# WQCG/blitzdg

Hardware: AMD Instinct MI355X
Metric: element-DOF updates/sec (sw2d RHS + LSERK4 stage, N=4, 1M tris) (higher is better)
Workload: dtype f64

## Files before the change

### blitzdg_amd/_capi.py

```python
import ctypes
import os
from ctypes import (POINTER, Structure, byref, c_char_p, c_double, c_float, c_int, c_size_t, c_uint,
                    c_ulonglong, c_void_p)

import numpy as np

_HERE = os.path.dirname(os.path.abspath(__file__))
os.environ.setdefault("HSA_ENABLE_IPC_MODE_LEGACY", "0")
LIB_PATH = os.environ.get("BDG_HIP_LIBRARY") or os.path.join(_HERE, "lib", "libblitzdg_hip.so")

BDG_OK, BDG_ERR_ARGUMENT, BDG_ERR_RUNTIME, BDG_ERR_HIP, BDG_ERR_UNSTABLE = 0, 1, 2, 3, 4
BDG_F64, BDG_I32 = 0, 1
BDG_SW2D_REORDER = 1
BDG_SW2D_NODAL_GEOMETRY = 2
BDG_SW2D_KEEP_ORDER = 4
BDG_SW2DQ_GENERAL_GEOMETRY = 1
(FIELD_STATS_SUM, FIELD_STATS_ETA_MAX, FIELD_STATS_H_MIN, FIELD_STATS_SPEED_MAX, FIELD_STATS_COS, FIELD_STATS_SIN) = range(6)

(MESH_VERTICES, MESH_ELEMENTS, MESH_ETOE, MESH_ETOF, MESH_BCTYPE, MESH_EPART, MESH_NPART) = range(7)
(TRI_R, TRI_S, TRI_X, TRI_Y, TRI_V, TRI_VINV, TRI_DR, TRI_DS, TRI_DRW, TRI_DSW, TRI_LIFT, TRI_FILTER,
 TRI_J, TRI_RX, TRI_RY, TRI_SX, TRI_SY, TRI_NX, TRI_NY, TRI_FSCALE, TRI_FMASK, TRI_FX, TRI_FY,
 TRI_VMAPM, TRI_VMAPP, TRI_MAPP, TRI_VMAPB, TRI_MAPB, TRI_GATHER, TRI_SCATTER) = range(30)
(GAUSS_NX, GAUSS_NY, GAUSS_SJ, GAUSS_J, GAUSS_RX, GAUSS_RY, GAUSS_SX, GAUSS_SY, GAUSS_X, GAUSS_Y, GAUSS_W,
 GAUSS_INTERP, GAUSS_MAPM, GAUSS_MAPP) = range(14)
(CUB_R, CUB_S, CUB_WEIGHTS, CUB_V, CUB_RX, CUB_RY, CUB_SX, CUB_SY, CUB_J, CUB_DR, CUB_DS, CUB_MM, CUB_MMCHOL,
 CUB_X, CUB_Y, CUB_W) = range(16)
(N1D_R, N1D_X, N1D_V, N1D_VINV, N1D_DR, N1D_LIFT, N1D_J, N1D_RX, N1D_NX, N1D_FMASK, N1D_FX,
 N1D_FSCALE, N1D_ETOV, N1D_ETOE, N1D_ETOF, N1D_VMAPM, N1D_VMAPP) = range(17)


class BdgError(RuntimeError):

    def __init__(self, code, message):
        super().__init__(message)
        self.code = code


class NumericalInstability(BdgError):
    """BDG_ERR_UNSTABLE: the reference drivers throw 'A numerical instability has occurred!'."""


class Table(Structure):
    _fields_ = [("data", c_void_p), ("rows", c_int), ("cols", c_int), ("dtype", c_int)]


class Sw2dDesc(Structure):
    _fields_ = [("order", c_int), ("num_elements", c_int),
                ("Dr", c_void_p), ("Ds", c_void_p), ("Lift", c_void_p), ("Filter", c_void_p),
                ("rx", c_void_p), ("sx", c_void_p), ("ry", c_void_p), ("sy", c_void_p),
                ("nx", c_void_p), ("ny", c_void_p), ("Fscale", c_void_p),
                ("vmapM", c_void_p), ("vmapP", c_void_p), ("mapW", c_void_p), ("num_wall", c_int),
                ("g", c_double), ("device", c_int), ("flags", c_int),
                ("num_fields", c_int), ("sources", c_int), ("zx", c_void_p), ("zy", c_void_p),
                ("coriolis", c_void_p), ("coriolis_const", c_double), ("drag", c_double)]

# ... 203 lines not shown
    "bdg_quadnodes_bed_slopes": (c_int, [_P, _P, _P, _P]),
    "bdg_quadnodes_sponge_coeff": (c_int, [_P, _P, c_int, c_double, c_double, _P]),
    "bdg_quadnodes_quadrature_weights": (c_int, [_P, _P]),
    "bdg_quadnodes_locate_points": (c_int, [_P, _P, _P, c_int, _P, _P, _P]),
    "bdg_quadnodes_lagrange_basis": (c_int, [_P, _P, c_int, _P]),
    "bdg_sw2dq_enable_monitor": (c_int, [_P, POINTER(Sw2dqMonitorDesc)]),
    "bdg_sw2dq_monitor_sample": (c_int, [_P]),
    "bdg_sw2dq_monitor_count": (c_int, [_P, POINTER(c_int)]),
    "bdg_sw2dq_monitor_read": (c_int, [_P, c_int, c_int, _P]),
    "bdg_sw2dq_monitor_width": (c_int, [_P, POINTER(c_int)]),
    "bdg_sw2dq_monitor_reset": (c_int, [_P]),
    "bdg_sw2dq_monitor_reduce": (c_int, [_P]),
    "bdg_quadnodes_drifter_tables": (c_int, [_P, _P, c_int, _P, _P, _P]),
    "bdg_sw2dq_enable_drifters": (c_int, [_P, POINTER(Sw2dqDrifterDesc)]),
    "bdg_sw2dq_drifters_advance": (c_int, [_P, c_double, c_int]),
    "bdg_sw2dq_drifters_time": (c_int, [_P, c_double, c_int, POINTER(c_float)]),
    "bdg_sw2dq_drifters_state": (c_int, [_P, _P, _P, _P, _P, _P, _P]),
    "bdg_sw2dq_drifters_count": (c_int, [_P, POINTER(c_int), POINTER(c_int)]),
    "bdg_sw2dq_drifters_read": (c_int, [_P, c_int, c_int, _P, _P, _P, _P]),
    "bdg_sw2dq_drifters_reset": (c_int, [_P]),
    "bdg_sw2d_step_lserk4": (c_int, [_P, c_double, c_int]),
    "bdg_sw2d_lserk4_stages": (c_int, [_P, c_double, c_int]),
    "bdg_sw2d_step_rk2": (c_int, [_P, c_double, c_int, c_int]),
    "bdg_sw2d_step_ssprk2": (c_int, [_P, c_double, c_int, c_int, c_double]),
    "bdg_sw2d_compute_dt": (c_int, [_P, c_double, POINTER(c_double), POINTER(c_double)]),
    "bdg_sw2d_run_adaptive": (c_int, [_P, c_double, c_double, c_int, c_int, POINTER(c_double),
                                      POINTER(c_double), POINTER(c_int)]),
    "bdg_sw2d_set_partition": (c_int, [_P, c_int, c_int, _P, c_int]),
    "bdg_sw2d_halo_doubles_per_element": (c_int, [_P]),
    "bdg_sw2d_halo_pack": (c_int, [_P, _P]),
    "bdg_sw2d_halo_unpack": (c_int, [_P, _P]),
    "bdg_sw2d_lserk4_stage_part": (c_int, [_P, c_double, c_int]),
    "bdg_comm_unique_id": (c_int, [_P, c_int]),
    "bdg_sw2d_comm_init": (c_int, [_P, c_int, c_int, _P, _P, _P, _P, _P, _P, c_int]),
    "bdg_sw2d_lserk4_stages_exchanged": (c_int, [_P, c_double, c_int]),
    "bdg_sw2d_step_rk2_exchanged": (c_int, [_P, c_double, c_int, c_int]),
    "bdg_sw2d_step_ssprk2_exchanged": (c_int, [_P, c_double, c_int, c_int, c_double]),
    "bdg_sw2d_local_peers": (c_int, [_P, c_int, _P, _P, _P, _P, _P, c_int]),
    "bdg_sw2d_group_lserk4_stages": (c_int, [POINTER(_P), c_int, c_double, c_int]),
    "bdg_sw2d_compute_dt_global": (c_int, [_P, c_double, POINTER(c_double), POINTER(c_double)]),
    "bdg_sw2d_allreduce_max": (c_int, [_P, c_double, POINTER(c_double)]),
    "bdg_sw2d_allreduce_sum": (c_int, [_P, c_double, POINTER(c_double)]),
    "bdg_sw2d_barrier": (c_int, [_P]),
    "bdg_sw2d_rhs_resident": (c_int, [_P, _P, _P, _P]),
    "bdg_sw2d_synchronize": (c_int, [_P]),
    "bdg_sw2d_time_lserk4_stages": (c_int, [_P, c_double, c_int, POINTER(c_float)]),
    "bdg_probe_stream_triad": (c_int, [c_int, c_size_t, c_int, POINTER(c_double)]),
    "bdg_sw2d_probe_stage_traffic": (c_int, [_P, c_int, POINTER(c_float)]),
    "bdg_sw2d_uses_affine_geometry": (c_int, [_P]),
    "bdg_sw2d_is_renumbered": (c_int, [_P]),
    "bdg_element_order": (c_int, [_P, c_int, c_int, _P]),
    "bdg_element_order_wanted": (c_int, [_P, c_int, c_int]),
    "bdg_sw2d_device_bytes": (c_size_t, [_P]),
    "bdg_sw2d_stream": (c_void_p, [_P]),
    "bdg_trinodes_quadrature_weights": (c_int, [_P, _P]),
    "bdg_trinodes_locate_points": (c_int, [_P, _P, _P, c_int, _P, _P, _P]),
    "bdg_trinodes_interpolation_rows": (c_int, [_P, _P, _P, c_int, _P]),
    "bdg_sw2d_enable_monitor": (c_int, [_P, POINTER(Sw2dMonitorDesc)]),
    "bdg_sw2d_monitor_sample": (c_int, [_P]),
    "bdg_sw2d_monitor_count": (c_int, [_P, POINTER(c_int)]),
    "bdg_sw2d_monitor_read": (c_int, [_P, c_int, c_int, _P]),
    "bdg_sw2d_monitor_width": (c_int, [_P, POINTER(c_int)]),
    "bdg_sw2d_monitor_reset": (c_int, [_P]),
    "bdg_sw2d_monitor_reduce": (c_int, [_P]),
    "bdg_sw2d_monitor_time": (c_int, [_P, c_int, POINTER(c_float)]),
    "bdg_trinodes_drifter_tables": (c_int, [_P, _P, c_int, _P, _P, _P, _P]),
    "bdg_sw2d_enable_drifters": (c_int, [_P, POINTER(Sw2dDrifterDesc)]),
    "bdg_sw2d_drifters_advance": (c_int, [_P, c_double, c_int]),
    "bdg_sw2d_drifters_time": (c_int, [_P, c_double, c_int, POINTER(c_float)]),
    "bdg_sw2d_drifters_state": (c_int, [_P, _P, _P, _P, _P, _P, _P]),
    "bdg_sw2d_drifters_count": (c_int, [_P, POINTER(c_int), POINTER(c_int)]),
    "bdg_sw2d_drifters_read": (c_int, [_P, c_int, c_int, _P, _P, _P, _P]),
    "bdg_sw2d_drifters_reset": (c_int, [_P]),
    **{f"{_abi}_{_name}": _sig for _abi in ("bdg_sw2d", "bdg_sw2dq") for _name, _sig in {
        "enable_field_stats": (c_int, [_P, POINTER(FieldStatsDesc)]),
        "field_stats_sample": (c_int, [_P]),
        "field_stats_count": (c_int, [_P, POINTER(c_int), POINTER(c_int)]),
        "field_stats_read": (c_int, [_P, c_int, c_int, _P]),
        "field_stats_samples": (c_int, [_P, c_int, c_int, _P]),
        "field_stats_reset": (c_int, [_P]),
        "field_stats_time": (c_int, [_P, c_int, POINTER(c_float)]),
    }.items()},
    "bdg_sw2d_curved_create": (c_int, [POINTER(Sw2dCurvedDesc), POINTER(_P)]),
    "bdg_sw2d_curved_plan": (c_int, [POINTER(Sw2dCurvedDesc), POINTER(c_int), c_int]),
    "bdg_sw2d_curved_destroy": (None, [_P]),
    "bdg_sw2d_curved_rhs": (c_int, [_P, _P, _P, _P, _P, _P, _P, _P, _P, c_int]),
    "bdg_sw2d_curved_set_state": (c_int, [_P, _P, _P, _P, _P]),
    "bdg_sw2d_curved_get_state": (c_int, [_P, _P, _P, _P, _P]),
    "bdg_sw2d_curved_step_rk2": (c_int, [_P, c_double, c_int, c_int]),
    "bdg_sw2d_curved_lserk4_stages": (c_int, [_P, c_double, c_int]),
    "bdg_sw2d_curved_time_rk2": (c_int, [_P, c_double, c_int, c_int, POINTER(c_float)]),
    "bdg_sw2d_curved_synchronize": (c_int, [_P]),
    "bdg_sw2d_curved_device_bytes": (c_size_t, [_P]),
    "bdg_sw2d_curved_bytes_per_element": (c_double, [_P]),
    "bdg_sw2d_curved_form": (c_int, [_P]),
    "bdg_sw2d_curved_kernel_info": (c_int, [_P, c_int, POINTER(c_int), c_int]),
    "bdg_sw2d_curved_get_elements": (c_int, [_P, c_int, c_int, c_int, POINTER(c_double)]),
    "bdg_sw2d_curved_set_elements": (c_int, [_P, c_int, c_int, c_int, POINTER(c_double)]),
    "bdg_sw2d_curved_rk2_phase": (c_int, [_P, c_double, c_int, c_int]),
    "bdg_sw2d_curved_set_partition": (c_int, [_P, c_int, c_int, _P, c_int]),
    "bdg_sw2d_curved_comm_init": (c_int, [_P, c_int, c_int, _P, _P, _P, _P, _P, _P, c_int]),
    "bdg_sw2d_curved_step_rk2_exchanged": (c_int, [_P, c_double, c_int, c_int]),
    "bdg_sw2d_curved_lserk4_stages_exchanged": (c_int, [_P, c_double, c_int]),
    "bdg_sw2d_curved_exchange": (c_int, [_P, c_int]),
    "bdg_sw2d_curved_barrier": (c_int, [_P]),
    "bdg_sw2d_curved_enable_driver": (c_int, [_P, POINTER(Sw2dCurvedDriverDesc)]),
# ... 55 lines not shown
```

### blitzdg_amd/csrc/hip/sw2d_affine_kernel.hpp

```cpp
#pragma once
#include "sw2d_kernels.hpp"

namespace bdg_dev {

template <int N>
struct AffineOps {
    using E = Elem<N>;
    static constexpr int OFF_D = 0;
    static constexpr int OFF_LIFT = 2 * E::Np * E::Np;
    static constexpr int DOUBLES = OFF_LIFT + E::NFN * E::Np;
};

__device__ __forceinline__ double fast_rcp(double x) {
    double r = __builtin_amdgcn_rcp(x);
    r = fma(fma(-x, r, 1.0), r, r);
    r = fma(fma(-x, r, 1.0), r, r);
    return r;
}

__device__ __forceinline__ double fast_sqrt(double x) {
    x = fmax(x, 1e-290);
    const double y = __builtin_amdgcn_rsq(x);
    double g = x * y, h = 0.5 * y;
    const double r = fma(-h, g, 0.5);
    g = fma(g, r, g);
    h = fma(h, r, h);
    g = fma(fma(-g, g, x), h, g);
    return g;
}

template <typename T>
__device__ __forceinline__ T ld_row(const T* row, unsigned byteOff) {
    return *reinterpret_cast<const T*>(reinterpret_cast<const char*>(row) + byteOff);
}
template <typename T>
__device__ __forceinline__ void st_row(T* row, unsigned byteOff, T v) {
    *reinterpret_cast<T*>(reinterpret_cast<char*>(row) + byteOff) = v;
}

struct PhysParams {
    const double* sx;
    const double* sy;
    const double* fcor;
    const double* fmat;
    double fconst, cd, slope, dragSign;
    const double* H;
    const int* obc;
    const double* lam;
    const double* spongeField;
    double tide;
};

template <int N>
__device__ __forceinline__ unsigned link_node(unsigned code, int n) {
    using E = Elem<N>;
    const bool rev = (code & 4u) != 0;
    const unsigned f = code & 3u;
    const unsigned m0 = rev ? E::fmask(0, N - n) : E::fmask(0, n);
    const unsigned m1 = rev ? E::fmask(1, N - n) : E::fmask(1, n);
    const unsigned m2 = rev ? E::fmask(2, N - n) : E::fmask(2, n);
    return f == 0u ? m0 : (f == 1u ? m1 : m2);
}

constexpr int STAGE_VMAP = -1;

template <int N, int MODE, int PHYS = 0, bool TRACER = false, bool SPONGE = false, int KIND = STAGE_VMAP>
__global__ __launch_bounds__(256) void sw2d_stage_affine_kernel(const StageParams p, const PhysParams ph) {
    using E = Elem<N>;
    constexpr int Np = E::Np, Nfp = E::Nfp, NFN = E::NFN;
    constexpr bool kLinks = KIND != STAGE_VMAP;
    static_assert(!kLinks || (MODE == MODE_LSERK && PHYS == 0 && !TRACER && !SPONGE), "face links: three-field LSERK stages");
    constexpr bool kReadRes = MODE == MODE_LSERK && KIND != STAGE_FIRST;
    constexpr bool kWriteRes = KIND != STAGE_LAST;

    const unsigned nwg = gridDim.x, xcd = blockIdx.x % 8u, q8 = nwg / 8u, r8 = nwg % 8u;
    const unsigned tile = (xcd < r8 ? xcd * (q8 + 1u) : r8 * (q8 + 1u) + (xcd - r8) * q8) + blockIdx.x / 8u;
    const unsigned k = static_cast<unsigned>(p.kbegin) + tile * blockDim.x + threadIdx.x;
    if (k >= static_cast<unsigned>(p.kend)) return;
    const unsigned k8 = k * 8u, k4 = k * 4u;

    const long long ld = p.ld, plane = static_cast<long long>(Np) * ld;
    const double* __restrict__ ops = p.opsAffine;
    const double* __restrict__ qin = p.qin;

    int idx[kLinks ? 1 : NFN];
    unsigned lnk[kLinks ? 3 : 1];
    if constexpr (kLinks) {
        const unsigned* __restrict__ fl = reinterpret_cast<const unsigned*>(p.faceLink);
#pragma unroll
        for (int f = 0; f < 3; ++f) lnk[f] = ld_row(fl + f * ld, k4);
    } else {
#pragma unroll
        for (int j = 0; j < NFN; ++j) idx[j] = ld_row(p.vmapP + j * ld, k4);
    }
    double h[Np], hu[Np], hv[Np], hN[TRACER ? Np : 1];
#pragma unroll
    for (int n = 0; n < Np; ++n) {
        h[n] = ld_row(qin + n * ld, k8);
        hu[n] = ld_row(qin + plane + n * ld, k8);
        hv[n] = ld_row(qin + 2 * plane + n * ld, k8);
        if constexpr (TRACER) hN[n] = ld_row(qin + 3 * plane + n * ld, k8);
    }
    const double* __restrict__ ag = p.ageo;
    const double rx = ld_row(ag, k8), sx = ld_row(ag + ld, k8), ry = ld_row(ag + 2 * ld, k8), sy = ld_row(ag + 3 * ld, k8);
    double fnx[3], fny[3], fsc[3];
#pragma unroll
    for (int f = 0; f < 3; ++f) {
        fnx[f] = ld_row(ag + (4 + f) * ld, k8);
        fny[f] = ld_row(ag + (7 + f) * ld, k8);
        fsc[f] = ld_row(ag + (10 + f) * ld, k8);
    }
    double ssx[PHYS != 0 ? Np : 1], ssy[PHYS != 0 ? Np : 1], sfc[PHYS != 0 ? Np : 1];
    if constexpr (PHYS != 0) {
#pragma unroll
        for (int i = 0; i < Np; ++i) { ssx[i] = 0.0; ssy[i] = 0.0; sfc[i] = ph.fconst; }
        if (ph.sx) {
#pragma unroll
            for (int i = 0; i < Np; ++i) ssx[i] = ld_row(ph.sx + i * ld, k8);
        }
        if (ph.sy) {
#pragma unroll
            for (int i = 0; i < Np; ++i) ssy[i] = ld_row(ph.sy + i * ld, k8);
        }
        if (ph.fcor) {
#pragma unroll
            for (int i = 0; i < Np; ++i) sfc[i] = ld_row(ph.fcor + i * ld, k8);
        }
    }
    __builtin_amdgcn_sched_barrier(0);
// ... 216 lines not shown
                n2 = a * old2[i] + dt * R2[i];
                n3 = a * old3[i] + dt * R3[i];
            } else if constexpr (kReadRes) {
                n1 = fma(dt, R1[i], a * old1[i]);
                n2 = fma(dt, R2[i], a * old2[i]);
                n3 = fma(dt, R3[i], a * old3[i]);
            } else {
                n1 = dt * R1[i];
                n2 = dt * R2[i];
                n3 = dt * R3[i];
            }
            if constexpr (kWriteRes) {
                st_row(rs + i * ld, k8, n1);
                st_row(rs + plane + i * ld, k8, n2);
                st_row(rs + 2 * plane + i * ld, k8, n3);
            }
            st_row(o + i * ld, k8, h[i] + b * n1);
            st_row(o + plane + i * ld, k8, hu[i] + b * n2);
            st_row(o + 2 * plane + i * ld, k8, hv[i] + b * n3);
            if constexpr (TRACER) {
                const double n4 = a * old4[i] + dt * R4[i];
                st_row(rs + 3 * plane + i * ld, k8, n4);
                st_row(o + 3 * plane + i * ld, k8, hN[i] + b * n4);
            }
        }
    } else {
        static_assert(!SPONGE || MODE == MODE_COMBINE, "the sponge follows a combine step");
        double* __restrict__ o = p.qout;
        const double a = p.ca, b = p.cb, c = p.cc;
        const double sg = p.sponge;
#pragma unroll
        for (int i = 0; i < Np; ++i) {
            const double v2 = a * old2[i] + b * hu[i] + c * R2[i], v3 = a * old3[i] + b * hv[i] + c * R3[i];
            st_row(o + i * ld, k8, a * old1[i] + b * h[i] + c * R1[i]);
            st_row(o + plane + i * ld, k8, SPONGE ? v2 / (1.0 + sg * v2 * v2) : v2);
            st_row(o + 2 * plane + i * ld, k8, SPONGE ? v3 / (1.0 + sg * v3 * v3) : v3);
        }
        if constexpr (TRACER) {
#pragma unroll
            for (int i = 0; i < Np; ++i) st_row(o + 3 * plane + i * ld, k8, a * old4[i] + b * hN[i] + c * R4[i]);
        }
    }
}

}

namespace bdg_dev {

template <int N, int MODE, int WAVES>
__global__ __launch_bounds__(256, WAVES) void sw2d_stage_affine_stream_kernel(const StageParams p) {
    using E = Elem<N>;
    constexpr int Np = E::Np, Nfp = E::Nfp;

    const unsigned nwg = gridDim.x, xcd = blockIdx.x % 8u, q8 = nwg / 8u, r8 = nwg % 8u;
    const unsigned tile = (xcd < r8 ? xcd * (q8 + 1u) : r8 * (q8 + 1u) + (xcd - r8) * q8) + blockIdx.x / 8u;
    const unsigned k = static_cast<unsigned>(p.kbegin) + tile * blockDim.x + threadIdx.x;
    if (k >= static_cast<unsigned>(p.kend)) return;
    const unsigned k8 = k * 8u, k4 = k * 4u;

    const long long ld = p.ld, plane = static_cast<long long>(Np) * ld;
    const double* __restrict__ ops = p.opsAffine;
    const double* __restrict__ qin = p.qin;
    const double* __restrict__ ag = p.ageo;
    const double g = p.g, halfg = 0.5 * p.g;

    double R1[Np], R2[Np], R3[Np];
#pragma unroll
    for (int i = 0; i < Np; ++i) R1[i] = R2[i] = R3[i] = 0.0;

    {
        const double rx = ld_row(ag, k8), sx = ld_row(ag + ld, k8), ry = ld_row(ag + 2 * ld, k8),
                     sy = ld_row(ag + 3 * ld, k8);
        constexpr int VCH = 5, NCH = (Np + VCH - 1) / VCH;
        double hc[2][VCH], huc[2][VCH], hvc[2][VCH];
#pragma unroll
        for (int t = 0; t < VCH; ++t)
            if (t < Np) {
                hc[0][t] = ld_row(qin + t * ld, k8);
                huc[0][t] = ld_row(qin + plane + t * ld, k8);
                hvc[0][t] = ld_row(qin + 2 * plane + t * ld, k8);
            }
#pragma unroll
        for (int c = 0; c < NCH; ++c) {
            const int cur = c & 1, nxt = cur ^ 1;
#pragma unroll
            for (int t = 0; t < VCH; ++t) {
                const int m = (c + 1) * VCH + t;
                if (m < Np) {
                    hc[nxt][t] = ld_row(qin + m * ld, k8);
                    huc[nxt][t] = ld_row(qin + plane + m * ld, k8);
                    hvc[nxt][t] = ld_row(qin + 2 * plane + m * ld, k8);
                }
            }
            __builtin_amdgcn_sched_barrier(0);
#pragma unroll
            for (int t = 0; t < VCH; ++t) {
                const int m = c * VCH + t;
                if (m < Np) {
                    const double h = hc[cur][t], hu = huc[cur][t], hv = hvc[cur][t];
                    const double r = fast_rcp(h);
                    const double u = hu * r, v = hv * r;
                    const double pr = halfg * h * h;
                    const double F2 = hu * u + pr, G2 = hu * v, G3 = hv * v + pr;
                    const double a1 = -(rx * hu + ry * hv), b1 = -(sx * hu + sy * hv);
                    const double a2 = -(rx * F2 + ry * G2), b2 = -(sx * F2 + sy * G2);
                    const double a3 = -(rx * G2 + ry * G3), b3 = -(sx * G2 + sy * G3);
#pragma unroll
                    for (int i = 0; i < Np; ++i) {
// ... 95 lines not shown
#pragma unroll
            for (int t = 0; t < CH; ++t) {
                const int i = i0 + t;
                if (i < Np) {
                    q1[t] = ld_row(qin + i * ld, k8);
                    q2[t] = ld_row(qin + plane + i * ld, k8);
                    q3[t] = ld_row(qin + 2 * plane + i * ld, k8);
                    o1[t] = ld_row(base2 + i * ld, k8);
                    o2[t] = ld_row(base2 + plane + i * ld, k8);
                    o3[t] = ld_row(base2 + 2 * plane + i * ld, k8);
                }
            }
            __builtin_amdgcn_sched_barrier(0);
#pragma unroll
            for (int t = 0; t < CH; ++t) {
                const int i = i0 + t;
                if (i < Np) {
                    if constexpr (MODE == MODE_LSERK) {
                        const double n1 = a * o1[t] + c * R1[i], n2 = a * o2[t] + c * R2[i], n3 = a * o3[t] + c * R3[i];
                        st_row(p.res + i * ld, k8, n1);
                        st_row(p.res + plane + i * ld, k8, n2);
                        st_row(p.res + 2 * plane + i * ld, k8, n3);
                        st_row(o + i * ld, k8, q1[t] + b * n1);
                        st_row(o + plane + i * ld, k8, q2[t] + b * n2);
                        st_row(o + 2 * plane + i * ld, k8, q3[t] + b * n3);
                    } else {
                        st_row(o + i * ld, k8, a * o1[t] + b * q1[t] + c * R1[i]);
                        st_row(o + plane + i * ld, k8, sponge_relax_no_test(a * o2[t] + b * q2[t] + c * R2[i], p.sponge));
                        st_row(o + 2 * plane + i * ld, k8, sponge_relax_no_test(a * o3[t] + b * q3[t] + c * R3[i], p.sponge));
                    }
                }
            }
            __builtin_amdgcn_sched_barrier(0);
        }
    }
}

}

namespace bdg_dev {

template <int N>
__device__ __forceinline__ int fmask_rt(int f, int n) {
    const int rs = n * (N + 1) - (n * (n - 1)) / 2;
    return f == 0 ? n : (f == 1 ? rs + (N - n) : rs);
}

template <int N, int MODE, int FIELDS>
__global__ __launch_bounds__(FIELDS == 3 ? 256 : 192, 2) void sw2d_stage_affine_rolled_kernel(const StageParams p) {
    using E = Elem<N>;
    constexpr int Np = E::Np, Nfp = E::Nfp;
    static_assert(FIELDS == 1 || FIELDS == 3, "FIELDS is 1 or 3");

    const unsigned nwg = gridDim.x, xcd = blockIdx.x % 8u, q8 = nwg / 8u, r8 = nwg % 8u;
    const unsigned tile = (xcd < r8 ? xcd * (q8 + 1u) : r8 * (q8 + 1u) + (xcd - r8) * q8) + blockIdx.x / 8u;
    const int c = FIELDS == 3 ? 0 : __builtin_amdgcn_readfirstlane(threadIdx.x >> 6);
    const unsigned k = static_cast<unsigned>(p.kbegin) +
                       (FIELDS == 3 ? tile * 256u + threadIdx.x : tile * 64u + (threadIdx.x & 63u));
    if (k >= static_cast<unsigned>(p.kend)) return;
    const unsigned k8 = k * 8u, k4 = k * 4u;

    const long long ld = p.ld, plane = static_cast<long long>(Np) * ld;
    const double* __restrict__ ops = p.opsAffine;
    const double* __restrict__ qin = p.qin;
    const double* __restrict__ ag = p.ageo;
    const double g = p.g, halfg = 0.5 * p.g;

    double R[FIELDS][Np];
#pragma unroll
    for (int q = 0; q < FIELDS; ++q)
#pragma unroll
        for (int i = 0; i < Np; ++i) R[q][i] = 0.0;

    {
        const double rx = ld_row(ag, k8), sx = ld_row(ag + ld, k8), ry = ld_row(ag + 2 * ld, k8),
                     sy = ld_row(ag + 3 * ld, k8);
        double h = ld_row(qin, k8), hu = ld_row(qin + plane, k8), hv = ld_row(qin + 2 * plane, k8);
#pragma unroll 1
        for (int m = 0; m < Np; ++m) {
            const int mn = m + 1 < Np ? m + 1 : m;
            const double hn = ld_row(qin + mn * ld, k8), hun = ld_row(qin + plane + mn * ld, k8),
                         hvn = ld_row(qin + 2 * plane + mn * ld, k8);
            const double r = fast_rcp(h);
            const double u = hu * r, v = hv * r;
            const double pr = halfg * h * h;
            const double F2 = hu * u + pr, G2 = hu * v, G3 = hv * v + pr;
            const double* __restrict__ row = ops + AffineOps<N>::OFF_D + 2 * m * Np;
            if constexpr (FIELDS == 3) {
                const double a1 = -(rx * hu + ry * hv), b1 = -(sx * hu + sy * hv);
                const double a2 = -(rx * F2 + ry * G2), b2 = -(sx * F2 + sy * G2);
                const double a3 = -(rx * G2 + ry * G3), b3 = -(sx * G2 + sy * G3);
#pragma unroll
                for (int i = 0; i < Np; ++i) {
                    const double dr = row[2 * i], ds = row[2 * i + 1];
                    R[0][i] = fma(ds, b1, fma(dr, a1, R[0][i]));
                    R[FIELDS - 2][i] = fma(ds, b2, fma(dr, a2, R[FIELDS - 2][i]));
                    R[FIELDS - 1][i] = fma(ds, b3, fma(dr, a3, R[FIELDS - 1][i]));
                }
            } else {
                const double F = c == 0 ? hu : (c == 1 ? F2 : G2);
                const double G = c == 0 ? hv : (c == 1 ? G2 : G3);
                const double a = -(rx * F + ry * G), b = -(sx * F + sy * G);
#pragma unroll
                for (int i = 0; i < Np; ++i) R[0][i] = fma(row[2 * i + 1], b, fma(row[2 * i], a, R[0][i]));
            }
            h = hn; hu = hun; hv = hvn;
        }
    }
// ... 101 lines not shown
```

### blitzdg_amd/csrc/hip/sw2d_affine_lean_kernel.hpp

```cpp
#pragma once
#include "sw2d_affine_kernel.hpp"

namespace bdg_dev {

template <int N>
__global__ __launch_bounds__(64, 2) void sw2d_stage_affine_lean_kernel(const StageParams p) {
    using E = Elem<N>;
    constexpr int Np = E::Np, Nfp = E::Nfp;

    const unsigned nwg = gridDim.x, xcd = blockIdx.x % 8u, q8 = nwg / 8u, r8 = nwg % 8u;
    const unsigned tile = (xcd < r8 ? xcd * (q8 + 1u) : r8 * (q8 + 1u) + (xcd - r8) * q8) + blockIdx.x / 8u;
    const unsigned k = static_cast<unsigned>(p.kbegin) + tile * blockDim.x + threadIdx.x;
    if (k >= static_cast<unsigned>(p.kend)) return;
    const unsigned k8 = k * 8u, k4 = k * 4u;

    const long long ld = p.ld, plane = static_cast<long long>(Np) * ld;
    const double* __restrict__ ops = p.opsAffine;
    const double* __restrict__ qin = p.qin;
    const double* __restrict__ ag = p.ageo;
    const double g = p.g, halfg = 0.5 * p.g;

    double h[Np], hu[Np], hv[Np];
#pragma unroll
    for (int n = 0; n < Np; ++n) {
        h[n] = ld_row(qin + n * ld, k8);
        hu[n] = ld_row(qin + plane + n * ld, k8);
        hv[n] = ld_row(qin + 2 * plane + n * ld, k8);
    }
    __builtin_amdgcn_sched_barrier(0);

    double R1[Np], R2[Np], R3[Np];
#pragma unroll
    for (int i = 0; i < Np; ++i) R1[i] = R2[i] = R3[i] = 0.0;

    {
        const double rx = ld_row(ag, k8), sx = ld_row(ag + ld, k8), ry = ld_row(ag + 2 * ld, k8), sy = ld_row(ag + 3 * ld, k8);
#pragma unroll
        for (int m = 0; m < Np; ++m) {
            const double r = fast_rcp(h[m]);
            const double u = hu[m] * r, v = hv[m] * r;
            const double pr = halfg * h[m] * h[m];
            const double F2 = hu[m] * u + pr, G2 = hu[m] * v, G3 = hv[m] * v + pr;
            const double a1 = -(rx * hu[m] + ry * hv[m]), b1 = -(sx * hu[m] + sy * hv[m]);
            const double a2 = -(rx * F2 + ry * G2), b2 = -(sx * F2 + sy * G2);
            const double a3 = -(rx * G2 + ry * G3), b3 = -(sx * G2 + sy * G3);
#pragma unroll
            for (int i = 0; i < Np; ++i) {
                const double dr = ops[AffineOps<N>::OFF_D + 2 * (m * Np + i)];
                R1[i] = fma(dr, a1, R1[i]);
                R2[i] = fma(dr, a2, R2[i]);
                R3[i] = fma(dr, a3, R3[i]);
            }
#pragma unroll
            for (int i = 0; i < Np; ++i) {
                const double ds = ops[AffineOps<N>::OFF_D + 2 * (m * Np + i) + 1];
                R1[i] = fma(ds, b1, R1[i]);
                R2[i] = fma(ds, b2, R2[i]);
                R3[i] = fma(ds, b3, R3[i]);
            }
        }
    }
    __builtin_amdgcn_sched_barrier(0);

#pragma unroll
// ... 89 lines not shown
```

### blitzdg_amd/csrc/hip/sw2d_affine_xchg_kernel.hpp

```cpp
#pragma once
#include "sw2d_affine_kernel.hpp"
#include "sw2d_mfma3_kernel.hpp"

namespace bdg_dev {

template <int N>
__global__ __launch_bounds__(64) void sw2d_stage_affine_xchg_kernel(const StageParams p, unsigned ldMagic) {
    using E = Elem<N>;
    constexpr int Np = E::Np, Nfp = E::Nfp, NFN = E::NFN;
    __shared__ double xs[3 * Np * 64];

    const unsigned nwg = gridDim.x, xcd = blockIdx.x % 8u, q8 = nwg / 8u, r8 = nwg % 8u;
    const unsigned tile = (xcd < r8 ? xcd * (q8 + 1u) : r8 * (q8 + 1u) + (xcd - r8) * q8) + blockIdx.x / 8u;
    const unsigned base = static_cast<unsigned>(p.kbegin) + tile * 64u, lane = threadIdx.x;
    const unsigned k = base + lane;
    if (k >= static_cast<unsigned>(p.kend)) return;
    const unsigned k8 = k * 8u, k4 = k * 4u;

    const long long ld = p.ld, plane = static_cast<long long>(Np) * ld;
    const unsigned ldu = static_cast<unsigned>(ld), planeBytes = static_cast<unsigned>(plane * 8);
    const double* __restrict__ ops = p.opsAffine;
    const double* __restrict__ qin = p.qin;
    const __amdgpu_buffer_rsrc_t rq = plane_rsrc(qin, 3u * planeBytes);

    int idx[NFN];
#pragma unroll
    for (int j = 0; j < NFN; ++j) idx[j] = ld_row(p.vmapP + j * ld, k4);
    double h[Np], hu[Np], hv[Np];
#pragma unroll
    for (int n = 0; n < Np; ++n) {
        h[n] = ld_row(qin + n * ld, k8);
        hu[n] = ld_row(qin + plane + n * ld, k8);
        hv[n] = ld_row(qin + 2 * plane + n * ld, k8);
    }
    const double* __restrict__ ag = p.ageo;
    const double rx = ld_row(ag, k8), sx = ld_row(ag + ld, k8), ry = ld_row(ag + 2 * ld, k8), sy = ld_row(ag + 3 * ld, k8);
    double fnx[3], fny[3], fsc[3];
#pragma unroll
    for (int f = 0; f < 3; ++f) {
        fnx[f] = ld_row(ag + (4 + f) * ld, k8);
        fny[f] = ld_row(ag + (7 + f) * ld, k8);
        fsc[f] = ld_row(ag + (10 + f) * ld, k8);
    }
    __builtin_amdgcn_sched_barrier(0);

    double hP[NFN], huP[NFN], hvP[NFN];
    unsigned ldsAt[NFN];
#pragma unroll
    for (int j = 0; j < NFN; ++j) {
        const unsigned o = static_cast<unsigned>(idx[j] < 0 ? -(idx[j] + 1) : idx[j]);
        unsigned nn = __umulhi(o, ldMagic);
        nn -= (nn * ldu > o) ? 1u : 0u;
        const unsigned kl = o - nn * ldu - base;
        const bool inwave = kl < 64u;
        ldsAt[j] = inwave ? nn * 64u + kl : 0xffffffffu;
        const unsigned o8 = inwave ? 0xfffffff8u : o * 8u;
        hP[j] = bld_f64(rq, o8, 0u);
        huP[j] = bld_f64(rq, o8, planeBytes);
        hvP[j] = bld_f64(rq, o8, 2u * planeBytes);
    }
    __builtin_amdgcn_sched_barrier(0);
#pragma unroll
    for (int n = 0; n < Np; ++n) {
        xs[n * 64 + lane] = h[n];
        xs[(Np + n) * 64 + lane] = hu[n];
        xs[(2 * Np + n) * 64 + lane] = hv[n];
// ... 121 lines not shown
```

### blitzdg_amd/csrc/hip/sw2d_device.hip

```cpp
#include "../host/capi_internal.hpp"
#include "../host/element_order.hpp"
#include "../host/parallel_for.hpp"
#include "blitzdg/LSERK4.hpp"
#include "run_records.hpp"
#include "sw2d_launch.hpp"
#include "sw2d_launch_host.hpp"
#include "sw2d_drifter_kernel.hpp"
#include <algorithm>
#include <atomic>
#include <cmath>
#include <cstdlib>
#include <cstring>
#include <limits>
#include <queue>
#include <stdexcept>
#include <string>
#include <vector>

namespace bdg_dev {

const KernelTable* kernel_table_order1();
const KernelTable* kernel_table_order2();
const KernelTable* kernel_table_order3();
const KernelTable* kernel_table_order4();
// ... 26 lines not shown
    for (int i = threadIdx.x; i < nblocks; i += blockDim.x) {
        const double x = part[2 * i], y = part[2 * i + 1];
        if (x != x || y != y) sBad = 1;
        a = fmax(a, x);
        b = fmax(b, y);
    }
    sA[threadIdx.x] = a;
    sB[threadIdx.x] = b;
    __syncthreads();
    for (int s = 128; s > 0; s >>= 1) {
        if (static_cast<int>(threadIdx.x) < s) {
            sA[threadIdx.x] = fmax(sA[threadIdx.x], sA[threadIdx.x + s]);
            sB[threadIdx.x] = fmax(sB[threadIdx.x], sB[threadIdx.x + s]);
        }
        __syncthreads();
    }
    if (threadIdx.x == 0) {
        const double nan = __builtin_nan("");
        out2[0] = sBad ? nan : sA[0];
        out2[1] = sBad ? nan : sB[0];
    }
}

template <typename T>
__global__ void scatter_rows_kernel(const T* __restrict__ src, T* __restrict__ dst, int rows, int K, long long ld,
                                    const int* __restrict__ perm) {
    const long long t = static_cast<long long>(blockIdx.x) * blockDim.x + threadIdx.x;
    if (t >= static_cast<long long>(rows) * K) return;
    const long long r = t / K, k = t % K;
    dst[r * ld + (perm ? perm[k] : k)] = src[t];
}

template <typename T>
__global__ void gather_rows_kernel(const T* __restrict__ src, T* __restrict__ dst, int rows, int K, long long ld,
                                   const int* __restrict__ perm) {
    const long long t = static_cast<long long>(blockIdx.x) * blockDim.x + threadIdx.x;
    if (t >= static_cast<long long>(rows) * K) return;
    const long long r = t / K, k = t % K;
    dst[t] = src[r * ld + (perm ? perm[k] : k)];
}

__global__ __launch_bounds__(256) void triad_kernel(double2* __restrict__ a, const double2* __restrict__ b,
                                                    const double2* __restrict__ c, double s, size_t n2) {
    const size_t stride = static_cast<size_t>(gridDim.x) * blockDim.x;
    for (size_t i = static_cast<size_t>(blockIdx.x) * blockDim.x + threadIdx.x; i < n2; i += stride) {
        const double2 x = b[i], y = c[i];
        a[i] = make_double2(x.x + s * y.x, x.y + s * y.y);
    }
}

__global__ __launch_bounds__(256) void stage_traffic_probe_kernel(const double* __restrict__ qin, double* __restrict__ qout,
                                                                 double* __restrict__ res, const double* __restrict__ ageo,
                                                                 const int* __restrict__ vmapP, int rows, int idxRows,
                                                                 long long ld, int K, int readRes, int writeRes) {
    const unsigned k = blockIdx.x * blockDim.x + threadIdx.x;
    if (k >= static_cast<unsigned>(K)) return;
    double acc = 0.0;
    for (int r = 0; r < 13; ++r) acc += ageo[r * ld + k];
    for (int r = 0; r < idxRows; ++r) acc += vmapP[r * ld + k];
    for (int r = 0; r < rows; ++r) {
        const double q = qin[r * ld + k], o = readRes ? res[r * ld + k] : 0.0;
        const double n = 0.5 * o + 1e-300 * (q + acc);
        if (writeRes) res[r * ld + k] = n;
        qout[r * ld + k] = q + 1e-300 * n;
    }
}

}

using bdg_detail::arg_error;
using bdg_detail::guard;
using bdg_detail::hip_error;
using bdg_detail::unstable_error;

using bdg_dev::DevBuf;
using bdg_dev::hipCheck;
using bdg_rccl::ncclCheck;
using bdg_rccl::rccl;

namespace {
std::vector<double> matmulHost(const double* A, const double* B, int n, int c);

namespace env {
int smallLaunchPinned() {
    static const int v = [] { const char* e = std::getenv("BDG_SW2D_SMALL_LAUNCH"); return e ? std::atoi(e) : -1; }();
    return v;
}
int interiorCapPinned() {
    static const int v = [] { const char* e = std::getenv("BDG_SW2D_INTERIOR_CAP"); return e ? std::atoi(e) : 0; }();
    return v;
}
bool extLaunch() {
    static const bool v = [] { const char* e = std::getenv("BDG_SW2D_EXT_LAUNCH"); return !e || e[0] != '0'; }();
    return v;
}
const char* affineVariantPin() { return std::getenv("BDG_SW2D_AFFINE_VARIANT"); }
bool nodalVector() { return std::getenv("BDG_SW2D_NODAL_VECTOR") != nullptr; }
bool fullStageTraffic() {
    const char* e = std::getenv("BDG_SW2D_FULL_STAGE_TRAFFIC");
    return e && e[0] != '0';
}
bool rolledSources() { return std::getenv("BDG_SW2D_ROLLED_SOURCES") != nullptr; }
bool eventFence() {
    const char* on = std::getenv("BDG_SW2D_EVENT_FENCE");
    const char* off = std::getenv("BDG_SW2D_EVENT_NOFENCE");
    return (on && on[0] == '1') || (off && off[0] == '0');
}
bool noCommWarmup() { return std::getenv("BDG_SW2D_NO_COMM_WARMUP") != nullptr; }
bool eventSync() {
    const char* e = std::getenv("BDG_SW2D_EVENT_SYNC");
    return e && e[0] != '0';
}
bool sourcesProduct() {
    const char* e = std::getenv("BDG_SW2D_SOURCES_PRODUCT");
    return e && e[0] != '0';
}
bool speedPass() { return std::getenv("BDG_SW2D_SPEED_PASS") != nullptr; }
bool tracerPass() { return std::getenv("BDG_SW2D_TRACER_PASS") != nullptr; }
bool sourcesTwoWave() { return std::getenv("BDG_SW2D_SOURCES_TWO_WAVE") != nullptr; }
bool haloKernels() { return std::getenv("BDG_SW2D_HALO_KERNELS") != nullptr; }
bool stripThroughput() { return std::getenv("BDG_SW2D_STRIP_THROUGHPUT") != nullptr; }
const char* haloVariant() { return std::getenv("BDG_SW2D_HALO_VARIANT"); }
}
}

struct bdg_sw2d {
    const bdg_dev::KernelTable* kt = nullptr;
    int N = 0, Np = 0, Nfp = 0, NFN = 0, K = 0, device = 0;
    long long ld = 0;
    double g = 9.81;
    bool hasFilter = false, hasH = false;
    hipStream_t stream = nullptr;
    size_t bytes = 0;
    DevBuf<double> qA, qB, res, aux, geo, fgeo, ops, Hbuf, stage, partials, red2;
    DevBuf<double> ageo, opsAffine, opsAffineFiltered;
    DevBuf<double> opsMfma, opsMfmaFiltered;
    DevBuf<double> opsMfma2, opsMfma2Filtered;
    DevBuf<double> opsMfma2Src, opsMfma2SrcFiltered;
    DevBuf<double> opsMfma2NodalFilter;
    bool mfmaSources = false;
    bool affine = false;
    bool nodalMfma = false;
    bool fastSources = false;
    static constexpr int kUnrolledSourcesMaxOrder = 4;
    DevBuf<double> filterT;
    int nf = 3;
    bool variantD = false;
    bdg_dev::VdParams vd{};
    DevBuf<double> zxBuf, zyBuf, fcorBuf, opsVd, opsVdFiltered;
    DevBuf<double> opsVn, filterRows, vnRaw;
    bool variantB = false;
    bdg_dev::VbParams vb{};
    DevBuf<double> HxBuf, HyBuf, spongeBuf, lamBuf, vbPartials;
    DevBuf<double> outM;
    DevBuf<int> obcBuf;
    double tideAmp = 0.0, tidePeriod = 1.0, tideRamp = 0.0;
    double timeNow = 0.0;
    bool lamExternal = false;
    DevBuf<double> lamPair;
    int lamSlot = 0;
    const double* lamStateFor = nullptr;
    double lamTideFor = 0.0;
    double nextEvalTime = 0.0;
    std::vector<double> hostDr, hostDs, hostLift, hostFilter, hostFDr, hostFDs, hostFLift;
    using AffineVariant = bdg_dev::AffineVariant;
    AffineVariant affineVariant = AffineVariant::Unrolled;
    bool variantForced = false;
    static constexpr int kSmallLaunch[6] = {0, 4000, 10000, 160000, 160000, 0};
    static constexpr int kInteriorGridCap = 244;
    DevBuf<int> vmapP, perm, istage, sendSlots, haloSendOf;
    DevBuf<int> faceLink;
    bool haloFusable = false;
    int numInterior = 0, numOwned = 0, numSend = 0;
    bdg_halo::Transport halo;
    hipEvent_t evA[2] = {nullptr, nullptr}, evB[2] = {nullptr, nullptr};
    hipEvent_t evPacked[2] = {nullptr, nullptr}, evCopied[2] = {nullptr, nullptr};
    bool localGroup = false;
    DevBuf<unsigned long long> syncBuf;
    unsigned long long expectRing = 0, expectStrip = 0;
    int ringBegin = 0;
    double* fscaleNodal = nullptr;
    double* qcur = nullptr;
    double* qalt = nullptr;
    long long stageCount = 0;
    double dtStage = 0.0;
    std::vector<int> permHost;
    struct Monitor : bdg_records::MonitorState {
        DevBuf<double> row;
        DevBuf<double> scratch;
    } mon;
    struct Drifters : bdg_records::DrifterState {
        DevBuf<double> vert, vinvT, jac;
        std::vector<int> callerOf;
    } drf;
    bdg_records::FieldStatsState fst;
    bool partitionSet = false;

    ~bdg_sw2d() {
        for (hipEvent_t e : {evA[0], evA[1], evB[0], evB[1], evPacked[0], evPacked[1], evCopied[0], evCopied[1]})
            if (e) (void)hipEventDestroy(e);
        if (stream) (void)hipStreamDestroy(stream);
    }

    void use() const { hipCheck(hipSetDevice(device), "hipSetDevice"); }
    size_t planeSize() const { return static_cast<size_t>(Np) * static_cast<size_t>(ld); }
    const int* permDev() const { return perm.p; }

    void uploadRows(const double* host, double* dev, int rows) {
        const size_t n = static_cast<size_t>(rows) * K;
        hipCheck(hipMemcpyAsync(stage.p, host, n * sizeof(double), hipMemcpyHostToDevice, stream), "H2D copy");
        const unsigned grid = static_cast<unsigned>((n + 255) / 256);
        hipLaunchKernelGGL((bdg_dev::scatter_rows_kernel<double>), dim3(grid), dim3(256), 0, stream, stage.p, dev, rows,
                           K, ld, permDev());
// ... 44 lines not shown
    }
    const double* stageOutputMatrix(const double* IM) {
        if (!IM) return nullptr;
        if (!outM.p) outM.alloc(static_cast<size_t>(Np) * Np, bytes);
        hipCheck(hipMemcpyAsync(outM.p, IM, outM.n * sizeof(double), hipMemcpyHostToDevice, stream), "H2D copy");
        return outM.p;
    }

    bdg_dev::StageParams baseParams() const {
        bdg_dev::StageParams p{};
        p.geo = geo.p;
        p.fgeo = fgeo.p;
        p.vmapP = vmapP.p;
        p.ops = ops.p;
        p.ageo = ageo.p;
        p.opsAffine = opsAffine.p;
        p.ld = ld;
        p.kbegin = 0;
        p.kend = numOwned;
        p.g = g;
        p.one = 1.0;
        return p;
    }

    double tideAt(double t) const {
        const double om = 2.0 * M_PI / tidePeriod;
        return tideAmp * std::cos(om * t) * 0.5 * (std::tanh(tideRamp * (t - tidePeriod)) + 1);
    }
    bdg_dev::PhysParams physB() const {
        bdg_dev::PhysParams ph{};
        ph.sx = vb.Hx; ph.sy = vb.Hy; ph.fconst = vb.fcor; ph.cd = vb.cd;
        ph.slope = 1.0; ph.dragSign = -1.0;
        ph.H = vb.H; ph.obc = vb.obc; ph.lam = lamBuf.p; ph.spongeField = vb.sponge; ph.tide = vb.tide;
        return ph;
    }
    bdg_dev::PhysParams physD() const {
        bdg_dev::PhysParams ph{};
        if (vd.sources) {
            ph.sx = vd.zx; ph.sy = vd.zy; ph.fcor = vd.fcor;
            ph.fconst = vd.fconst; ph.cd = vd.cd;
            ph.slope = -1.0; ph.dragSign = 1.0;
        }
        return ph;
    }
    bool variantBStateOnce() const { return kt->mfma3SrcFields >= 3 && !env::sourcesTwoWave() && fitsOneDescriptor(3); }
    static bool srcIdentity(bool filter) { return !filter && !env::sourcesProduct(); }
    bool fitsOneDescriptor(int fields) const { return bdg_dev::fitsOneDescriptor(fields, Np, ld); }
    int interiorGridCap() const {
        if (env::interiorCapPinned() > 0) return env::interiorCapPinned();
        if (N < 5) return kInteriorGridCap;
        return N >= 8 ? 244 : 248;
    }

    void launchStage(int mode, bool filter, bdg_dev::StageParams& p, const char* what, hipStream_t on = nullptr) {
        if (filter && !hasFilter) throw arg_error("filter requested but the solver was created without a Filter matrix");
        hipStream_t st = on ? on : stream;
        AffineVariant variant = affineVariant;
        const int smallPinned = env::smallLaunchPinned();
        const int smallLaunch = (smallPinned >= 0 && p.kbegin == 0) ? smallPinned : kSmallLaunch[N];
        if (!variantForced && affine && N <= 5 && p.kend - p.kbegin < smallLaunch) variant = AffineVariant::Mfma;
        if (p.syncSignal && !(affine && !variantB && !variantD && (variant == AffineVariant::Mfma || variant == AffineVariant::Mfma3)))
            throw std::logic_error("in-kernel stage dependencies were requested for a launch whose kernel has no SYNC instance");
        if (!affine && (variantB || variantD)) {
            buildNodalVariantOps();
            const double* filt = filter ? filterRows.p : nullptr;
            if (variantB) {
                vb.tide = tideAt(timeNow);
                vb.lam = lamBuf.p;
                vb.lamNext = nullptr;
                lamStateFor = nullptr;
                hipCheck(kt->stageVn(mode, true, p, vd, vb, opsVn.p, filt, vnRaw.p, vbPartials.p, lamBuf.p, !lamExternal, st), what);
            } else {
                bdg_dev::VdParams v = vd;
                v.cbase = 0;
                hipCheck(kt->stageVn(mode, false, p, v, vb, opsVn.p, filt, vnRaw.p, nullptr, nullptr, false, st), what);
            }
        } else if (variantB) {
            using bdg_dev::SrcForm;
            using bdg_dev::VbStage;
            vb.tide = tideAt(timeNow);
            enum class Speed { Reduced, Reused, OwnPass };
            const bool whole = p.kbegin == 0 && p.kend == numOwned;
            const bool reusable = fastSources && whole && lamStateFor == p.qin && lamTideFor == vb.tide && !env::speedPass();
            const Speed speed = lamExternal ? Speed::Reduced : (reusable ? Speed::Reused : Speed::OwnPass);
            const bool ownPass = speed == Speed::OwnPass;
            const int cur = lamSlot, nxt = lamSlot ^ 1;
            vb.lam = speed == Speed::Reused ? lamPair.p + cur : lamBuf.p;
            vb.lamNext = nullptr;
            lamStateFor = nullptr;
            if (fastSources && !lamExternal && whole && mode != bdg_dev::MODE_RHS) {
                hipCheck(hipMemsetAsync(lamPair.p + nxt, 0, sizeof(double), st), "hipMemset");
                vb.lamNext = reinterpret_cast<unsigned long long*>(lamPair.p + nxt);
                vb.tideNext = tideAt(nextEvalTime);
                lamStateFor = p.qout;
                lamTideFor = vb.tideNext;
                lamSlot = nxt;
            }
            if (fastSources) {
                p.opsAffine = opsAffine.p;
                hipCheck(kt->stageVb(mode, p, vb, vbPartials.p, lamBuf.p, ownPass, VbStage::Unrolled, filter ? filterT.p : nullptr, st), what);
            } else if (mfmaSources) {
                if (ownPass) hipCheck(kt->stageVb(mode, p, vb, vbPartials.p, lamBuf.p, true, VbStage::None, nullptr, st), what);
                p.opsAffine = filter ? opsMfma2SrcFiltered.p : opsMfma2Src.p;
                hipCheck(kt->stageMfma2Src(mode, p, physB(), variantBStateOnce() ? SrcForm::OnceVariantB : SrcForm::VariantB, srcIdentity(filter), st), what);
            } else {
                p.opsAffine = filter ? opsVdFiltered.p : opsVd.p;
                hipCheck(kt->stageVb(mode, p, vb, vbPartials.p, lamBuf.p, ownPass, VbStage::Rolled, nullptr, st), what);
            }
        } else if (variantD && fastSources) {
            bdg_dev::PhysParams ph = physD();
            ph.fmat = filter ? filterT.p : nullptr;
            p.opsAffine = opsAffine.p;
            if (nf == 4 && !env::tracerPass()) {
                hipCheck(kt->stageAffineSrc(mode, p, ph, true, st), what);
            } else {
                hipCheck(kt->stageAffineSrc(mode, p, ph, false, st), what);
                if (nf == 4) {
                    p.opsAffine = filter ? opsAffineFiltered.p : opsAffine.p;
                    hipCheck(kt->stageTracer(mode, p, st), what);
                }
            }
        } else if (variantD && mfmaSources) {
            using bdg_dev::SrcForm;
            const bdg_dev::PhysParams ph = physD();
            const bool identity = srcIdentity(filter);
            p.opsAffine = filter ? opsMfma2SrcFiltered.p : opsMfma2Src.p;
            const bool stateOnceSrc = !env::sourcesTwoWave();
            if (stateOnceSrc && kt->mfma3SrcFields >= nf && !env::tracerPass() && fitsOneDescriptor(nf)) {
                hipCheck(kt->stageMfma2Src(mode, p, ph, nf == 4 ? SrcForm::OnceSourcesTracer : SrcForm::OnceSources, identity, st), what);
            } else if (stateOnceSrc && kt->mfma3TracerPhase && nf == 4 && !env::tracerPass() && fitsOneDescriptor(4)) {
                hipCheck(kt->stageMfma2Src(mode, p, ph, SrcForm::OnceTracerPhase, identity, st), what);
            } else if (stateOnceSrc && kt->mfma3SrcFields == 3 && nf == 4 && fitsOneDescriptor(3)) {
                hipCheck(kt->stageMfma2Src(mode, p, ph, SrcForm::OnceSources, identity, st), what);
                p.opsAffine = filter ? opsMfma2Filtered.p : opsMfma2.p;
                hipCheck(kt->stageMfma2Src(mode, p, ph, SrcForm::TracerPass, false, st), what);
            } else if (nf == 4 && kt->mfmaMT <= 2 && !env::tracerPass()) {
                hipCheck(kt->stageMfma2Src(mode, p, ph, SrcForm::SourcesTracer, false, st), what);
            } else {
                hipCheck(kt->stageMfma2Src(mode, p, ph, SrcForm::Sources, false, st), what);
                if (nf == 4) {
                    p.opsAffine = filter ? opsMfma2Filtered.p : opsMfma2.p;
                    hipCheck(kt->stageMfma2Src(mode, p, ph, SrcForm::TracerPass, false, st), what);
                }
            }
        } else if (variantD) {
            p.opsAffine = filter ? opsVdFiltered.p : opsVd.p;
            hipCheck(kt->stageVd(mode, p, vd, st), what);
        } else if (affine && variant == AffineVariant::Mfma) {
            p.opsAffine = filter ? opsMfmaFiltered.p : opsMfma.p;
            hipCheck(kt->stageMfma(mode, p, st), what);
        } else if (affine && variant == AffineVariant::Mfma3) {
            p.opsAffine = filter ? opsMfma2Filtered.p : opsMfma2.p;
            hipCheck(kt->stageMfma3(mode, p, st), what);
        } else if (affine && variant == AffineVariant::Mfma2) {
            p.opsAffine = filter ? opsMfma2Filtered.p : opsMfma2.p;
            hipCheck(kt->stageMfma2(mode, p, st), what);
        } else if (affine) {
            p.opsAffine = filter ? opsAffineFiltered.p : opsAffine.p;
            hipCheck(kt->stageAffine(mode, variant, p, st), what);
        } else if (nodalMfma) {
            p.opsAffine = filter ? opsMfma2NodalFilter.p : opsMfma2.p;
            hipCheck(kt->stageMfma3Nodal(mode, filter, p, st), what);
        } else {
            hipCheck(kt->stage(mode, filter, p, st), what);
        }
    }

    void launchRhs(const double* qin, double* out, bool filter) {
        bdg_dev::StageParams p = baseParams();
        p.qin = qin;
        p.rhs = out;
        launchStage(bdg_dev::MODE_RHS, filter, p, "sw2d stage kernel <RHS>");
    }

    int lserkStageParams(bdg_dev::StageParams& p, hipEvent_t done, bool* recorded) const {
        const int s = static_cast<int>(stageCount % blitzdg::LSERK4::numStages);
        const bool extLaunch = env::extLaunch();
        if (done && extLaunch) { p.stopEvent = done; p.stopEventUsed = recorded; }
        p.qin = qcur;
        p.qout = qalt;
        p.res = res.p;
        p.ca = blitzdg::LSERK4::rk4a[s];
        p.cb = blitzdg::LSERK4::rk4b[s];
        p.cc = dtStage;
        return s;
    }
    void lserkStageAdvance(int s) {
        std::swap(qcur, qalt);
        ++stageCount;
        if (s == blitzdg::LSERK4::numStages - 1) timeNow += dtStage;
    }
    void launchLserkStage(int part = 2, hipStream_t on = nullptr, bool advance = true, hipEvent_t done = nullptr, bool flagSync = false) {
        bdg_dev::StageParams p = baseParams();
        bool recorded = false;
        unsigned signals = 0;
        if (flagSync && part == 0) {
            p.syncWait = syncBuf.p + 1; p.syncWaitValue = expectStrip;
            p.syncSignal = syncBuf.p; p.syncError = reinterpret_cast<unsigned int*>(syncBuf.p + 2);
            p.syncFirstTile = ringBegin / 16;
            p.syncSignalsOut = &signals;
        }
        const int s = lserkStageParams(p, done, &recorded);
        if (part == 0) {
            p.kend = numInterior;
            p.gridCap = interiorGridCap();
        }
        if (part == 1) p.kbegin = numInterior;
        const bool lastOfStep = s == blitzdg::LSERK4::numStages - 1;
        p.faceLink = faceLink.p;
        p.stageKind = p.ca == 0.0 ? bdg_dev::STAGE_FIRST : (lastOfStep ? bdg_dev::STAGE_LAST : bdg_dev::STAGE_MID);
        nextEvalTime = lastOfStep ? timeNow + dtStage : timeNow;
        launchStage(bdg_dev::MODE_LSERK, false, p, "sw2d stage kernel <LSERK>", on);
        expectRing += signals;
        if (done && !recorded) hipCheck(hipEventRecord(done, on ? on : stream), "hipEventRecord");
        if (part != 0 && advance) lserkStageAdvance(s);
    }

    void launchPack(double* buf, hipStream_t on = nullptr, const double* state = nullptr) {
        bdg_halo::pack(state ? state : qcur, ld, nf * Np, sendSlots.p, numSend, buf, on ? on : stream);
    }
    void launchUnpack(const double* buf, hipStream_t on = nullptr, double* state = nullptr) {
        bdg_halo::unpack(state ? state : qcur, ld, nf * Np, numOwned, K - numOwned, buf, on ? on : stream);
    }

    void exchangeGhostsOf(double* state) {
        if (!halo.comm) throw arg_error("no communicator: call bdg_sw2d_comm_init first");
        launchPack(halo.sendBuf.p, stream, state);
        halo.sendRecv(stream, nf * Np);
        launchUnpack(halo.recvBuf.p, stream, state);
    }
    void globalSpeedOf(const double* state) {
        bdg_dev::StageParams p = baseParams();
        p.qin = state;
        vb.tide = tideAt(timeNow);
        vb.lam = lamBuf.p;
        hipCheck(kt->stageVb(bdg_dev::MODE_RHS, p, vb, vbPartials.p, lamBuf.p, true, bdg_dev::VbStage::None, nullptr, stream), "sw2d_vb_speed_kernel");
        if (halo.comm && halo.world > 1)
            ncclCheck(rccl().AllReduce(lamBuf.p, lamBuf.p, 1, ncclDouble, ncclMax, halo.comm, stream), "ncclAllReduce");
    }
    template <typename Fn>
    void evaluateExchanged(double* state, Fn&& fn) {
        exchangeGhostsOf(state);
        if (variantB) {
            globalSpeedOf(state);
            lamExternal = true;
        }
        try {
            fn();
        } catch (...) {
            lamExternal = false;
            throw;
        }
        lamExternal = false;
    }

    bool halosFold() const {
        if (!haloFusable || !affine || variantB || variantD || variantForced || env::haloKernels()) return false;
        return N >= 5 || numOwned - numInterior < kSmallLaunch[N];
    }
    bool flagSyncUsable() const {
        if (env::eventSync() || !syncBuf.p || !halosFold()) return false;
        if (env::stripThroughput() || env::haloVariant()) return false;
        if (N >= 5) return affineVariant == AffineVariant::Mfma3 && (numOwned - numInterior + 15) / 16 <= 1024;
        const int smallPinned = env::smallLaunchPinned();
        return numInterior > 0 && affineVariant == AffineVariant::Unrolled && numInterior < (smallPinned >= 0 ? smallPinned : kSmallLaunch[N]);
// ... 368 lines not shown

    const size_t plane3 = static_cast<size_t>(s->nf) * s->planeSize();
    s->qA.alloc(plane3, s->bytes);
    s->qB.alloc(plane3, s->bytes);
    s->res.alloc(plane3, s->bytes);
    s->aux.alloc(plane3, s->bytes);
    const size_t fplane = static_cast<size_t>(NFN) * ld;
    if (!s->affine) {
        s->geo.alloc(4 * s->planeSize(), s->bytes);
        s->fgeo.alloc(3 * fplane, s->bytes);
        s->ops.alloc(kt->ldsDoubles, s->bytes);
    } else {
        s->fgeo.alloc(fplane, s->bytes);
    }
    s->fscaleNodal = s->affine ? s->fgeo.p : s->fgeo.p + 2 * fplane;
    s->vmapP.alloc(static_cast<size_t>(NFN) * ld, s->bytes);
    s->stage.alloc(static_cast<size_t>(std::max(Np, NFN)) * K, s->bytes);
    s->istage.alloc(static_cast<size_t>(NFN) * K, s->bytes);
    s->partials.alloc(2 * static_cast<size_t>((K + 255) / 256), s->bytes);
    s->red2.alloc(2, s->bytes);
    if (!s->permHost.empty()) s->perm.upload(s->permHost, s->bytes, "perm upload");
    for (auto* b : {&s->qA, &s->qB, &s->res, &s->aux, &s->geo, &s->fgeo})
        if (b->p) hipCheck(hipMemsetAsync(b->p, 0, b->n * sizeof(double), s->stream), "hipMemset");
    hipCheck(hipMemsetAsync(s->vmapP.p, 0, s->vmapP.n * sizeof(int), s->stream), "hipMemset");
    s->qcur = s->qA.p;
    s->qalt = s->qB.p;

    s->hasFilter = d.Filter != nullptr;
    if (!s->affine && kt->ldsDoubles > 0) {
        std::vector<double> img(kt->ldsDoubles, 0.0);
        for (int i = 0; i < Np * Np; ++i) {
            img[2 * i] = d.Dr[i];
            img[2 * i + 1] = d.Ds[i];
        }
        std::copy(d.Lift, d.Lift + static_cast<size_t>(Np) * NFN, img.begin() + 2 * Np * Np);
        if (d.Filter) std::copy(d.Filter, d.Filter + static_cast<size_t>(Np) * Np, img.begin() + 2 * Np * Np + Np * NFN);
        hipCheck(hipMemcpyAsync(s->ops.p, img.data(), img.size() * sizeof(double), hipMemcpyHostToDevice, s->stream),
                 "ops upload");
        hipCheck(hipStreamSynchronize(s->stream), "ops sync");
    }

    if (!s->affine) {
        const size_t pl = s->planeSize();
        s->uploadRows(d.rx, s->geo.p, Np);
        s->uploadRows(d.sx, s->geo.p + pl, Np);
        s->uploadRows(d.ry, s->geo.p + 2 * pl, Np);
        s->uploadRows(d.sy, s->geo.p + 3 * pl, Np);
        s->uploadRows(d.nx, s->fgeo.p, NFN);
        s->uploadRows(d.ny, s->fgeo.p + fplane, NFN);
    }
    s->uploadRows(d.Fscale, s->fscaleNodal, NFN);

    s->affineVariant = s->N <= 4 ? bdg_dev::AffineVariant::Unrolled : bdg_dev::AffineVariant::Mfma3;
    if (const char* e = env::affineVariantPin()) {
        const int v = std::atoi(e);
        if (v >= 0 && v <= 9) {
            s->affineVariant = static_cast<bdg_dev::AffineVariant>(v);
            s->variantForced = true;
        }
    }
    s->hostDr.assign(d.Dr, d.Dr + static_cast<size_t>(Np) * Np);
    s->hostDs.assign(d.Ds, d.Ds + static_cast<size_t>(Np) * Np);
    s->hostLift.assign(d.Lift, d.Lift + static_cast<size_t>(Np) * NFN);
    if (d.Filter) {
        s->hostFilter.assign(d.Filter, d.Filter + static_cast<size_t>(Np) * Np);
        s->hostFDr = matmulHost(d.Filter, d.Dr, Np, Np);
        s->hostFDs = matmulHost(d.Filter, d.Ds, Np, Np);
        s->hostFLift = matmulHost(d.Filter, d.Lift, Np, NFN);
    }
    auto mfmaImage = [&](const double* Dr, const double* Ds, const double* Lift) {
        const int MT = kt->mfmaMT, KV = kt->mfmaKV, KS = kt->mfmaKS;
        std::vector<double> img(static_cast<size_t>(kt->mfmaOpsDoubles), 0.0);
        auto fill = [&](size_t off, const double* A, int cols, int KT) {
            for (int r = 0; r < MT; ++r)
                for (int t = 0; t < KT; ++t)
                    for (int l = 0; l < 64; ++l) {
                        const int i = 16 * r + (l & 15), k = 4 * t + (l >> 4);
                        if (i < Np && k < cols) img[off + (static_cast<size_t>(r) * KT + t) * 64 + l] = A[i * cols + k];
                    }
        };
        fill(0, Dr, Np, KV);
        fill(static_cast<size_t>(MT) * KV * 64, Ds, Np, KV);
        fill(static_cast<size_t>(2) * MT * KV * 64, Lift, NFN, KS);
        return img;
    };
    auto mfma2Image = [&](const double* Dr, const double* Ds, const double* Lift) {
        const int MT = kt->mfmaMT, KV = kt->mfmaKV, KF = kt->mfma2KF;
        std::vector<double> img(static_cast<size_t>(kt->mfma2OpsDoubles), 0.0);
        const std::vector<double> first = mfmaImage(Dr, Ds, Lift);
        std::copy(first.begin(), first.begin() + static_cast<size_t>(2) * MT * KV * 64, img.begin());
        const size_t off = static_cast<size_t>(2) * MT * KV * 64;
        for (int r = 0; r < MT; ++r)
            for (int f = 0; f < 3; ++f)
                for (int tf = 0; tf < KF; ++tf)
                    for (int l = 0; l < 64; ++l) {
                        const int i = 16 * r + (l & 15), n = 4 * tf + (l >> 4);
                        if (i < Np && n < Nfp)
                            img[off + ((static_cast<size_t>(r) * 3 + f) * KF + tf) * 64 + l] = Lift[i * NFN + f * Nfp + n];
                    }
        return img;
    };
    if (s->nodalMfma) {
        const std::vector<double> img2 = mfma2Image(d.Dr, d.Ds, d.Lift);
        s->opsMfma2.upload(img2, s->bytes, "mfma2 ops upload");
        if (d.Filter) {
            std::vector<double> imgF = img2;
// ... 1034 lines not shown
int bdg_sw2d_field_stats_samples(const bdg_sw2d* s, int first, int count, double* rows) {
    return guard([&] {
        requireStatsOn(s, "bdg_sw2d_field_stats_samples");
        s->fst.samples("bdg_sw2d_field_stats_samples", first, count, rows);
    });
}

int bdg_sw2d_field_stats_reset(bdg_sw2d* s) {
    return guard([&] {
        requireStatsOn(s, "bdg_sw2d_field_stats_reset");
        s->use();
        s->fst.reset(s->stream);
    });
}

int bdg_sw2d_field_stats_time(bdg_sw2d* s, int count, float* ms) {
    return guard([&] {
        requireStatsOn(s, "bdg_sw2d_field_stats_time");
        if (count < 1 || !ms) throw arg_error("bdg_sw2d_field_stats_time: bad argument");
        s->use();
        *ms = s->fst.time(s->statsView(), count, s->bytes, s->stream);
    });
}

int bdg_probe_stream_triad(int device, size_t bytes_per_array, int repeats, double* gbps) {
    return guard([&] {
        if (!gbps || repeats < 1 || bytes_per_array < (1u << 20)) throw arg_error("bdg_probe_stream_triad: bad argument");
        hipCheck(hipSetDevice(device), "hipSetDevice");
        const size_t n2 = bytes_per_array / sizeof(double2);
        size_t total = 0;
        DevBuf<double> a, b, c;
        a.alloc(2 * n2, total); b.alloc(2 * n2, total); c.alloc(2 * n2, total);
        hipCheck(hipMemset(a.p, 0, 2 * n2 * sizeof(double)), "hipMemset");
        hipCheck(hipMemset(b.p, 0, 2 * n2 * sizeof(double)), "hipMemset");
        hipCheck(hipMemset(c.p, 0, 2 * n2 * sizeof(double)), "hipMemset");
        auto launch = [&] {
            hipLaunchKernelGGL(bdg_dev::triad_kernel, dim3(256 * 8), dim3(256), 0, nullptr, reinterpret_cast<double2*>(a.p),
                               reinterpret_cast<const double2*>(b.p), reinterpret_cast<const double2*>(c.p), 0.5, n2);
        };
        launch();
        const float ms = bdg_dev::timePerRun(nullptr, repeats, launch);
        *gbps = 3.0 * static_cast<double>(n2) * sizeof(double2) / (ms * 1e-3) / 1e9;
    });
}

int bdg_sw2d_probe_stage_traffic(bdg_sw2d* s, int repeats, float* ms_per_launch) {
    return guard([&] {
        requireSolver(s, "bdg_sw2d_probe_stage_traffic");
        if (!ms_per_launch || repeats < 1) throw arg_error("bdg_sw2d_probe_stage_traffic: bad argument");
        if (!s->affine) throw arg_error("bdg_sw2d_probe_stage_traffic: affine geometry only");
        s->use();
        const unsigned grid = static_cast<unsigned>((s->K + 255) / 256);
        const bool links = s->faceLink.p != nullptr;
        auto launch = [&](int stage) {
            const int last = blitzdg::LSERK4::numStages - 1;
            hipLaunchKernelGGL(bdg_dev::stage_traffic_probe_kernel, dim3(grid), dim3(256), 0, s->stream, s->qcur, s->qalt,
                               s->aux.p, s->ageo.p, links ? s->faceLink.p : s->vmapP.p, 3 * s->Np, links ? 3 : s->NFN, s->ld,
                               s->K, !links || stage != 0 ? 1 : 0, !links || stage != last ? 1 : 0);
        };
        launch(1);
        int i = 0;
        *ms_per_launch = bdg_dev::timePerRun(s->stream, repeats, [&] { launch(i++ % blitzdg::LSERK4::numStages); });
    });
}

int bdg_sw2d_uses_affine_geometry(const bdg_sw2d* s) { return s ? (s->affine ? 1 : 0) : -1; }
int bdg_sw2d_is_renumbered(const bdg_sw2d* s) { return s ? (s->permHost.empty() ? 0 : 1) : -1; }

size_t bdg_sw2d_device_bytes(const bdg_sw2d* s) { return s ? s->bytes : 0; }
void* bdg_sw2d_stream(bdg_sw2d* s) { return s ? static_cast<void*>(s->stream) : nullptr; }

}
```

### blitzdg_amd/csrc/hip/sw2d_kernels.hpp

```cpp
#pragma once
#include <hip/hip_runtime.h>

namespace bdg_dev {

template <int N>
struct Elem {
    static constexpr int Np = (N + 1) * (N + 2) / 2;
    static constexpr int Nfp = N + 1;
    static constexpr int NFN = 3 * Nfp;
    __host__ __device__ static constexpr int rowStart(int j) { return j * (N + 1) - j * (j - 1) / 2; }
    __host__ __device__ static constexpr int fmask(int f, int n) {
        return f == 0 ? n : (f == 1 ? rowStart(n) + (N - n) : rowStart(n));
    }
    static constexpr int OFF_D = 0;
    static constexpr int OFF_LIFT = 2 * Np * Np;
    static constexpr int OFF_FILT = OFF_LIFT + Np * NFN;
    static constexpr int LDS_DOUBLES = OFF_FILT + Np * Np;
};

struct FaceLink {
    static constexpr unsigned SLOT_MASK = 0x0FFFFFFFu;
    static constexpr int FACE_SHIFT = 28;
    static constexpr unsigned REVERSED = 1u << 30;
    static constexpr unsigned WALL = 1u << 31;
    __host__ __device__ static constexpr unsigned make(unsigned slot, unsigned face, bool reversed, bool wall) {
        return slot | (face << FACE_SHIFT) | (reversed ? REVERSED : 0u) | (wall ? WALL : 0u);
    }
};

enum StageKind {
    STAGE_FIRST = 0,
    STAGE_MID = 1,
    STAGE_LAST = 2
};

enum StageMode {
    MODE_RHS = 0,
    MODE_LSERK = 1,
    MODE_COMBINE = 2
};

struct StageParams {
    const double* qin;
    const double* qbase;
    double* qout;
    double* res;
    double* rhs;
    const double* geo;
    const double* fgeo;
    const int* vmapP;
    const int* faceLink;
    int stageKind;
    const double* ops;
    const double* ageo;
    const double* opsAffine;
    long long ld;
    int kbegin, kend;
    double g;
    double ca, cb, cc;
    double one;
    double sponge;
    const double* haloRecv;
    double* haloSend;
    const int* haloSendOf;
    int haloOwned;
    int haloRows;
    int gridCap;
    int tileInterleave;
    int stagger;
    unsigned long long* phaseClock;
    const unsigned long long* syncWait;
    unsigned long long syncWaitValue;
    unsigned long long* syncSignal;
    unsigned int* syncError;
    int syncFirstTile;
    unsigned int* syncSignalsOut;
    hipEvent_t stopEvent;
    bool* stopEventUsed;
};

constexpr unsigned kSyncSpinLimit = 1u << 21;
__device__ __forceinline__ void sync_wait(const unsigned long long* ctr, unsigned long long want, unsigned int* err) {
    unsigned spins = 0;
    while (__hip_atomic_load(ctr, __ATOMIC_RELAXED, __HIP_MEMORY_SCOPE_AGENT) < want) {
        __builtin_amdgcn_s_sleep(4);
        if (++spins > kSyncSpinLimit) {
            if (err) __hip_atomic_store(err, 1u, __ATOMIC_RELAXED, __HIP_MEMORY_SCOPE_AGENT);
            break;
        }
    }
    __builtin_amdgcn_fence(__ATOMIC_ACQUIRE, "agent");
}
__device__ __forceinline__ void sync_signal_wave(unsigned long long* ctr) {
    asm volatile("s_waitcnt vmcnt(0)" ::: "memory");
    if ((threadIdx.x & 63u) == 0u) __hip_atomic_fetch_add(ctr, 1ull, __ATOMIC_RELAXED, __HIP_MEMORY_SCOPE_AGENT);
}
__device__ __forceinline__ void sync_signal_workgroup(unsigned long long* ctr) {
    asm volatile("s_waitcnt vmcnt(0)" ::: "memory");
    __syncthreads();
    if (threadIdx.x == 0u) __hip_atomic_fetch_add(ctr, 1ull, __ATOMIC_RELAXED, __HIP_MEMORY_SCOPE_AGENT);
}
__device__ __forceinline__ void st_row_wt(double* row, unsigned byteOff, double v) {
    __hip_atomic_store(reinterpret_cast<double*>(reinterpret_cast<char*>(row) + byteOff), v, __ATOMIC_RELAXED, __HIP_MEMORY_SCOPE_AGENT);
}

__device__ __forceinline__ double sponge_relax(double x, double sigma) {
    return sigma != 0.0 ? x / (1.0 + sigma * x * x) : x;
}
__device__ __forceinline__ double sponge_relax_no_test(double x, double sigma) { return x / (1.0 + sigma * x * x); }

template <int N, int MODE, bool FILTER>
__global__ __launch_bounds__(256) void sw2d_stage_kernel(const StageParams p) {
    using E = Elem<N>;
    constexpr int Np = E::Np, Nfp = E::Nfp, NFN = E::NFN;
    __shared__ double sOps[E::LDS_DOUBLES];
    for (int t = threadIdx.x; t < E::LDS_DOUBLES; t += blockDim.x) sOps[t] = p.ops[t];
    __syncthreads();

    const unsigned nwg = gridDim.x, xcd = blockIdx.x % 8u, q8 = nwg / 8u, r8 = nwg % 8u;
    const unsigned tile = (xcd < r8 ? xcd * (q8 + 1u) : r8 * (q8 + 1u) + (xcd - r8) * q8) + blockIdx.x / 8u;
    const long long k = p.kbegin + static_cast<long long>(tile) * blockDim.x + threadIdx.x;
    if (k >= p.kend) return;

    const long long ld = p.ld, plane = static_cast<long long>(Np) * ld;
    const double* __restrict__ qh = p.qin + k;
    const double* __restrict__ qhu = qh + plane;
    const double* __restrict__ qhv = qhu + plane;

    double h[Np], hu[Np], hv[Np];
    int idx[NFN];
#pragma unroll
    for (int j = 0; j < NFN; ++j) idx[j] = p.vmapP[j * ld + k];
#pragma unroll
    for (int n = 0; n < Np; ++n) {
        h[n] = qh[n * ld];
        hu[n] = qhu[n * ld];
        hv[n] = qhv[n * ld];
    }
    double hP[NFN], huP[NFN], hvP[NFN];
#pragma unroll
    for (int j = 0; j < NFN; ++j) {
        const int o = idx[j] < 0 ? -(idx[j] + 1) : idx[j];
        hP[j] = p.qin[o];
        huP[j] = p.qin[plane + o];
        hvP[j] = p.qin[2 * plane + o];
    }

    const double g = p.g, halfg = 0.5 * p.g;
    double u[Np], v[Np], F2[Np], G2[Np], G3[Np];
#pragma unroll
    for (int n = 0; n < Np; ++n) {
        u[n] = hu[n] / h[n];
        v[n] = hv[n] / h[n];
        const double pr = halfg * h[n] * h[n];
        F2[n] = hu[n] * u[n] + pr;
        G2[n] = hu[n] * v[n];
        G3[n] = hv[n] * v[n] + pr;
    }

    double s1[NFN], s2[NFN], s3[NFN];
    const double* __restrict__ fg = p.fgeo + k;
    const long long fplane = static_cast<long long>(NFN) * ld;
#pragma unroll
    for (int f = 0; f < 3; ++f) {
        double lam = 0.0;
        double dh[Nfp], dhu[Nfp], dhv[Nfp], e1[Nfp], e2[Nfp], e3[Nfp];
#pragma unroll
        for (int n = 0; n < Nfp; ++n) {
            const int j = f * Nfp + n, m = E::fmask(f, n);
            const double nxj = fg[j * ld], nyj = fg[fplane + j * ld];
            const double hM = h[m], huM = hu[m], hvM = hv[m];
            double hPj = hP[j], huPj = huP[j], hvPj = hvP[j];
            if (idx[j] < 0) {
// ... 210 lines not shown
```

### blitzdg_amd/csrc/hip/sw2d_mfma3_kernel.hpp

```cpp
#pragma once
#include "sw2d_mfma_kernel.hpp"

namespace bdg_dev {

typedef unsigned int bdg_u32x2 __attribute__((ext_vector_type(2)));
__device__ __forceinline__ __amdgpu_buffer_rsrc_t plane_rsrc(const void* base, unsigned bytes) {
    return __builtin_amdgcn_make_buffer_rsrc(const_cast<void*>(base), 0, bytes, 0x00020000);
}
__device__ __forceinline__ double bld_f64(__amdgpu_buffer_rsrc_t r, unsigned voff, unsigned soff) {
    return __builtin_bit_cast(double, __builtin_amdgcn_raw_buffer_load_b64(r, voff, soff, 0));
}
__device__ __forceinline__ int bld_i32(__amdgpu_buffer_rsrc_t r, unsigned voff, unsigned soff) {
    return static_cast<int>(__builtin_amdgcn_raw_buffer_load_b32(r, voff, soff, 0));
}
__device__ __forceinline__ void bst_f64(__amdgpu_buffer_rsrc_t r, unsigned voff, unsigned soff, double v) {
    __builtin_amdgcn_raw_buffer_store_b64(__builtin_bit_cast(bdg_u32x2, v), r, voff, soff, 0);
}
__device__ __forceinline__ void bst_f64_wt(__amdgpu_buffer_rsrc_t r, unsigned voff, unsigned soff, double v) {
    __builtin_amdgcn_raw_buffer_store_b64(__builtin_bit_cast(bdg_u32x2, v), r, voff, soff, 16);
}

__device__ __forceinline__ mfma_acc_t mfma_zero() {
    mfma_acc_t z{0.0, 0.0, 0.0, 0.0};
    asm volatile("" : "+v"(z));
    return z;
}

template <int Np, int KV>
__device__ __forceinline__ unsigned row_voffset(int t, unsigned q, unsigned v8) {
    if constexpr (Np % 4 != 0) {
        if (t == KV - 1) return (4 * (KV - 1) + static_cast<int>(q) < Np) ? v8 : 0xfffffff8u;
    }
    return v8;
}

template <int N>
struct Mfma3Lds {
    using O = MfmaOps2<N>;
    static constexpr int TILE_DOUBLES = 3 * Elem<N>::Np * 16;
    static constexpr int DOUBLES = O::DOUBLES + 4 * TILE_DOUBLES;
};

template <int N, int MODE, bool HALO = false, bool NODAL = false, bool NFILT = false, bool SYNC = false>
__global__ __launch_bounds__(256, 1) void sw2d_stage_mfma3_kernel(const StageParams p) {
    static_assert(!HALO || MODE == MODE_LSERK, "halo staging is folded into LSERK stages only");
    static_assert(!SYNC || (MODE == MODE_LSERK && !HALO && !NODAL), "in-kernel stage dependencies: interior launches of LSERK stages");
    static_assert(!(HALO && NODAL), "partitioned runs use the straight-sided form");
    static_assert(NODAL || !NFILT, "straight-sided elements take the filter through pre-multiplied operators");
    using E = Elem<N>;
    using O = MfmaOps2<N>;
    constexpr int Np = E::Np, Nfp = E::Nfp, MT = O::MT, KV = O::KV, KF = O::KF;

    constexpr int IMAGE = O::DOUBLES + (NFILT ? MT * KV * 64 : 0);
    constexpr bool PF = !((NODAL || HALO) && MT >= 3 && KV >= 12);
    extern __shared__ double sOps[];
    stage_image<IMAGE, 256>(sOps, p.opsAffine);
    __syncthreads();
    const int sBase = IMAGE + static_cast<int>(threadIdx.x >> 6) * Mfma3Lds<N>::TILE_DOUBLES + static_cast<int>(threadIdx.x & 15u);

    const unsigned lane = threadIdx.x & 63u, q = lane >> 4, j = lane & 15u;
    const unsigned nwg = gridDim.x, xcd = blockIdx.x % 8u, q8 = nwg / 8u, r8 = nwg % 8u;
    const unsigned blk = (xcd < r8 ? xcd * (q8 + 1u) : r8 * (q8 + 1u) + (xcd - r8) * q8) + blockIdx.x / 8u;
    const unsigned wave = blk * 4u + (threadIdx.x >> 6), nwaves = nwg * 4u;
    const unsigned ntiles = (static_cast<unsigned>(p.kend - p.kbegin) + 15u) / 16u;
    const unsigned perWave = (ntiles + nwaves - 1u) / nwaves;
    unsigned tileEnd = min(ntiles, (wave + 1u) * perWave), tileStep = 1u;
    unsigned tile = wave * perWave;
    if (p.tileInterleave) {
        const unsigned wgHere = (nwg + 7u - xcd) / 8u, wgBefore = blk - blockIdx.x / 8u;
        tile = ntiles * wgBefore / nwg + (blockIdx.x / 8u) * 4u + (threadIdx.x >> 6);
        tileEnd = ntiles * (wgBefore + wgHere) / nwg;
        tileStep = wgHere * 4u;
    }
    if (tile >= tileEnd) return;

    const long long ld = p.ld, plane = static_cast<long long>(Np) * ld;
    const double g = p.g, halfg = 0.5 * p.g;
    const unsigned kLast = static_cast<unsigned>(p.kend) - 1u;
    const unsigned planeBytes = static_cast<unsigned>(plane * 8), ld8 = static_cast<unsigned>(ld) * 8u, ld4 = static_cast<unsigned>(ld) * 4u;
    __amdgpu_buffer_rsrc_t rq[3], rold[3], rout[3], rres[3];
#pragma unroll
    for (int c = 0; c < 3; ++c) {
        rq[c] = plane_rsrc(p.qin + c * plane, planeBytes);
        rold[c] = plane_rsrc((MODE == MODE_LSERK ? p.res : (MODE == MODE_COMBINE ? p.qbase : p.qin)) + c * plane, planeBytes);
        rout[c] = plane_rsrc((MODE == MODE_RHS ? p.rhs : p.qout) + c * plane, planeBytes);
        rres[c] = plane_rsrc((MODE == MODE_LSERK ? p.res : p.qin) + c * plane, planeBytes);
    }
    const __amdgpu_buffer_rsrc_t rgeo = plane_rsrc(NODAL ? p.geo : p.ageo, NODAL ? planeBytes : 13u * ld8),
                                 ridx = plane_rsrc(p.vmapP, 3u * Nfp * ld4);
    __amdgpu_buffer_rsrc_t rmet[4], rfg[3];
#pragma unroll
    for (int i = 0; i < 4; ++i) rmet[i] = plane_rsrc(NODAL ? p.geo + i * plane : p.ageo, NODAL ? planeBytes : 8u);
#pragma unroll
    for (int i = 0; i < 3; ++i)
        rfg[i] = plane_rsrc(NODAL ? p.fgeo + static_cast<long long>(i) * 3 * Nfp * ld : p.ageo, NODAL ? 3u * Nfp * ld8 : 8u);
    const __amdgpu_buffer_rsrc_t rrecv = plane_rsrc(HALO ? p.haloRecv : p.ageo, 0xffffffffu);

    auto elementOf = [&](unsigned tl, bool& live) {
        const unsigned kTrue = static_cast<unsigned>(p.kbegin) + tl * 16u + j;
        live = kTrue <= kLast;
        return live ? kTrue : kLast;
    };
    auto loadStateRow = [&](unsigned kk, int t, double (&qs)[3][KV]) {
        const unsigned v8 = (q * static_cast<unsigned>(ld) + kk) * 8u;
#pragma unroll
        for (int c = 0; c < 3; ++c) qs[c][t] = bld_f64(rq[c], row_voffset<Np, KV>(t, q, v8), static_cast<unsigned>(4 * t) * ld8);
    };
    auto loadIndices = [&](unsigned kk, int (&ix)[3][KF]) {
        const unsigned v4 = (q * static_cast<unsigned>(ld) + kk) * 4u;
#pragma unroll
        for (int f = 0; f < 3; ++f)
#pragma unroll
            for (int tf = 0; tf < KF; ++tf)
                ix[f][tf] = bld_i32(ridx, (4 * tf + static_cast<int>(q) < Nfp) ? v4 : 0xfffffffcu, static_cast<unsigned>(f * Nfp + 4 * tf) * ld4);
    };
    auto loadGeometry = [&](unsigned kk, double (&gg)[13]) {
        if constexpr (!NODAL) {
#pragma unroll
            for (int i = 0; i < 13; ++i) gg[i] = bld_f64(rgeo, kk * 8u, static_cast<unsigned>(i) * ld8);
        }
    };
    auto loadMetricRow = [&](unsigned kk, int t, double (&mm)[4]) {
        const unsigned v8 = (q * static_cast<unsigned>(ld) + kk) * 8u;
#pragma unroll
        for (int i = 0; i < 4; ++i) mm[i] = bld_f64(rmet[i], row_voffset<Np, KV>(t, q, v8), static_cast<unsigned>(4 * t) * ld8);
    };
    auto loadFaceGeometry = [&](int f, unsigned kk, double (&fx)[3][KF], double (&fy)[3][KF], double (&fs)[3][KF]) {
        const unsigned v8 = (q * static_cast<unsigned>(ld) + kk) * 8u;
#pragma unroll
        for (int tf = 0; tf < KF; ++tf) {
            const unsigned vo = (4 * tf + static_cast<int>(q) < Nfp) ? v8 : 0xfffffff8u;
            const unsigned so = static_cast<unsigned>(f * Nfp + 4 * tf) * ld8;
            fx[f][tf] = bld_f64(rfg[0], vo, so);
            fy[f][tf] = bld_f64(rfg[1], vo, so);
            fs[f][tf] = bld_f64(rfg[2], vo, so);
        }
    };
    auto loadTraces = [&](int f, const int (&ix)[3][KF], double (&a)[3][KF], double (&b)[3][KF], double (&c3)[3][KF]) {
#pragma unroll
        for (int tf = 0; tf < KF; ++tf) {
            const int n = 4 * tf + static_cast<int>(q);
            const int id = n < Nfp ? ix[f][tf] : 0;
            const unsigned idp = static_cast<unsigned>(id < 0 ? -(id + 1) : id), o8 = idp * 8u;
            if constexpr (HALO) {
                const unsigned row = idp / static_cast<unsigned>(ld), slot = idp - row * static_cast<unsigned>(ld);
                if (slot >= static_cast<unsigned>(p.haloOwned)) {
                    const unsigned rec8 = ((slot - static_cast<unsigned>(p.haloOwned)) * static_cast<unsigned>(p.haloRows) + row) * 8u;
                    a[f][tf] = bld_f64(rrecv, rec8, 0u);
                    b[f][tf] = bld_f64(rrecv, rec8, static_cast<unsigned>(Np) * 8u);
                    c3[f][tf] = bld_f64(rrecv, rec8, static_cast<unsigned>(2 * Np) * 8u);
                    continue;
                }
// ... 583 lines not shown
```

### blitzdg_amd/csrc/hip/sw2d_mfma3src_kernel.hpp

```cpp
#pragma once
#include "sw2d_mfma3_kernel.hpp"

namespace bdg_dev {

template <int N, bool TRACER>
struct Mfma3SrcLds {
    using O = MfmaOps2<N>;
    static constexpr int NF = TRACER ? 4 : 3;
    static constexpr int IMAGE = O::DOUBLES + O::MT * O::KV * 64;
    static constexpr int TILE_DOUBLES = NF * Elem<N>::Np * 16;
    static constexpr int DOUBLES = IMAGE + 4 * TILE_DOUBLES;
};

template <int N, int MODE, bool TRACER, int PHYS = 1, bool TPHASE = false, bool IDF = false>
__global__ __launch_bounds__(256, 1) void sw2d_stage_mfma3src_kernel(const StageParams p, const PhysParams ph) {
    static_assert(PHYS == 1 || (PHYS == 2 && !TRACER), "variant B has three fields");
    static_assert(!TPHASE || (PHYS == 1 && !TRACER), "the tracer phase follows the three-field form of variants C / D");
    using E = Elem<N>;
    using O = MfmaOps2<N>;
    using L = Mfma3SrcLds<N, TRACER || TPHASE>;
    constexpr int Np = E::Np, Nfp = E::Nfp, MT = O::MT, KV = O::KV, KF = O::KF, NF = TRACER ? 4 : 3;
    constexpr int NFD = (TRACER || TPHASE) ? 4 : 3;
    constexpr int IMAGE = L::IMAGE, OFF_F = O::DOUBLES;
    constexpr bool PF = KV < 12;
    constexpr bool PF2 = TPHASE && !PF;

    extern __shared__ double sOps[];
    stage_image<IDF ? O::DOUBLES : IMAGE, 256>(sOps, p.opsAffine);
    __syncthreads();
    const int sBase = IMAGE + static_cast<int>(threadIdx.x >> 6) * L::TILE_DOUBLES + static_cast<int>(threadIdx.x & 15u);

    const unsigned lane = threadIdx.x & 63u, q = lane >> 4, j = lane & 15u;
    const unsigned nwg = gridDim.x, xcd = blockIdx.x % 8u, q8 = nwg / 8u, r8 = nwg % 8u;
    const unsigned blk = (xcd < r8 ? xcd * (q8 + 1u) : r8 * (q8 + 1u) + (xcd - r8) * q8) + blockIdx.x / 8u;
    const unsigned ntiles = (static_cast<unsigned>(p.kend - p.kbegin) + 15u) / 16u;
    const unsigned wgHere = (nwg + 7u - xcd) / 8u, wgBefore = blk - blockIdx.x / 8u;
    unsigned tile = ntiles * wgBefore / nwg + (blockIdx.x / 8u) * 4u + (threadIdx.x >> 6);
    const unsigned tileEnd = ntiles * (wgBefore + wgHere) / nwg, tileStep = wgHere * 4u;
    if (tile >= tileEnd) return;

    const long long ld = p.ld, plane = static_cast<long long>(Np) * ld;
    const double g = p.g, halfg = 0.5 * p.g;
    const unsigned kLast = static_cast<unsigned>(p.kend) - 1u;
    const unsigned planeBytes = static_cast<unsigned>(plane * 8), ld8 = static_cast<unsigned>(ld) * 8u, ld4 = static_cast<unsigned>(ld) * 4u;
    const __amdgpu_buffer_rsrc_t rq = plane_rsrc(p.qin, NFD * planeBytes),
                                 rold = plane_rsrc(MODE == MODE_LSERK ? p.res : (MODE == MODE_COMBINE ? p.qbase : p.qin), NFD * planeBytes),
                                 rout = plane_rsrc(MODE == MODE_RHS ? p.rhs : p.qout, NFD * planeBytes),
                                 rgeo = plane_rsrc(p.ageo, 13u * ld8), ridx = plane_rsrc(p.vmapP, 3u * Nfp * ld4),
                                 rsx = plane_rsrc(ph.sx ? ph.sx : p.ageo, ph.sx ? planeBytes : 0u),
                                 rsy = plane_rsrc(ph.sy ? ph.sy : p.ageo, ph.sy ? planeBytes : 0u),
                                 rfc = plane_rsrc(ph.fcor ? ph.fcor : p.ageo, ph.fcor ? planeBytes : 0u);
    const __amdgpu_buffer_rsrc_t rH = plane_rsrc(PHYS == 2 ? ph.H : p.ageo, PHYS == 2 ? planeBytes : 0u),
                                 robc = plane_rsrc(PHYS == 2 ? static_cast<const void*>(ph.obc) : static_cast<const void*>(p.ageo), PHYS == 2 ? ld4 : 0u),
                                 rsp = plane_rsrc((PHYS == 2 && ph.spongeField) ? ph.spongeField : p.ageo,
                                                  (PHYS == 2 && ph.spongeField) ? planeBytes : 0u);
    const bool hasSp = PHYS == 2 && ph.spongeField != nullptr;
    const double lamGlobal = PHYS == 2 ? *ph.lam : 0.0, tide = ph.tide;
    const bool hasF = ph.fcor != nullptr;
    const double cd = ph.cd, slope = ph.slope, dragSign = ph.dragSign, fconst = ph.fconst;

    auto elementOf = [&](unsigned tl, bool& live) {
        const unsigned kTrue = static_cast<unsigned>(p.kbegin) + tl * 16u + j;
        live = kTrue <= kLast;
        return live ? kTrue : kLast;
    };
    auto loadStateRow = [&](unsigned kk, int t, double (&qs)[NF][KV], double (&src)[3][KV]) {
        const unsigned vo = row_voffset<Np, KV>(t, q, (q * static_cast<unsigned>(ld) + kk) * 8u), so = static_cast<unsigned>(4 * t) * ld8;
#pragma unroll
        for (int c = 0; c < NF; ++c) qs[c][t] = bld_f64(rq, vo, static_cast<unsigned>(c) * planeBytes + so);
        src[0][t] = bld_f64(rsx, vo, so);
        src[1][t] = bld_f64(rsy, vo, so);
        src[2][t] = bld_f64(rfc, vo, so);
    };
    auto loadStateOnly = [&](unsigned kk, int t, double (&qs)[NF][KV]) {
        const unsigned vo = row_voffset<Np, KV>(t, q, (q * static_cast<unsigned>(ld) + kk) * 8u), so = static_cast<unsigned>(4 * t) * ld8;
#pragma unroll
        for (int c = 0; c < NF; ++c) qs[c][t] = bld_f64(rq, vo, static_cast<unsigned>(c) * planeBytes + so);
    };
    auto loadSourceRow = [&](unsigned kk, int t, double (&src)[3][KV]) {
        const unsigned vo = row_voffset<Np, KV>(t, q, (q * static_cast<unsigned>(ld) + kk) * 8u), so = static_cast<unsigned>(4 * t) * ld8;
        src[0][t] = bld_f64(rsx, vo, so);
        src[1][t] = bld_f64(rsy, vo, so);
        src[2][t] = bld_f64(rfc, vo, so);
    };
    auto loadIndices = [&](unsigned kk, int (&ix)[3][KF]) {
        const unsigned v4 = (q * static_cast<unsigned>(ld) + kk) * 4u;
#pragma unroll
        for (int f = 0; f < 3; ++f)
#pragma unroll
            for (int tf = 0; tf < KF; ++tf)
                ix[f][tf] = bld_i32(ridx, (4 * tf + static_cast<int>(q) < Nfp) ? v4 : 0xfffffffcu, static_cast<unsigned>(f * Nfp + 4 * tf) * ld4);
    };
    auto loadGeometry = [&](unsigned kk, double (&gg)[13]) {
#pragma unroll
        for (int i = 0; i < 13; ++i) gg[i] = bld_f64(rgeo, kk * 8u, static_cast<unsigned>(i) * ld8);
    };
    auto loadTraces = [&](int f, unsigned kk, const int (&ix)[3][KF], double (&tr)[NF][3][KF], double (&dep)[2][3][KF]) {
#pragma unroll
        for (int tf = 0; tf < KF; ++tf) {
            const int n = 4 * tf + static_cast<int>(q);
            const int id = n < Nfp ? ix[f][tf] : 0;
            const unsigned o8 = static_cast<unsigned>(id < 0 ? -(id + 1) : id) * 8u;
#pragma unroll
            for (int c = 0; c < NF; ++c) tr[c][f][tf] = bld_f64(rq, o8, static_cast<unsigned>(c) * planeBytes);
            if constexpr (PHYS == 2) {
                const int m = n < Nfp ? fmask_rt<N>(f, n) : 0;
                dep[0][f][tf] = bld_f64(rH, (static_cast<unsigned>(m) * static_cast<unsigned>(ld) + kk) * 8u, 0u);
                dep[1][f][tf] = bld_f64(rH, o8, 0u);
            }
        }
    };

    bool live;
    unsigned k = elementOf(tile, live);
    double qB[NF][KV], srcB[3][KV], geo[13], trP[NF][3][KF], depP[2][3][KF];
// ... 418 lines not shown
```

### blitzdg_amd/csrc/hip/sw2d_mfma_kernel.hpp

```cpp
#pragma once
#include "sw2d_affine_kernel.hpp"

namespace bdg_dev {

typedef double bdg_f64x2 __attribute__((ext_vector_type(2)));
template <int COUNT, int THREADS>
__device__ __attribute__((noinline)) void stage_image(double* __restrict__ lds, const double* __restrict__ src) {
    static_assert(COUNT % 2 == 0, "operator images are whole 64-double tiles");
    constexpr int PAIRS = COUNT / 2, STEPS = (PAIRS + THREADS - 1) / THREADS;
    const bdg_f64x2* __restrict__ s2 = reinterpret_cast<const bdg_f64x2*>(src);
    bdg_f64x2* __restrict__ d2 = reinterpret_cast<bdg_f64x2*>(lds);
    bdg_f64x2 v[STEPS];
#pragma unroll
    for (int i = 0; i < STEPS; ++i) {
        const int at = i * THREADS + static_cast<int>(threadIdx.x);
        if (at < PAIRS) v[i] = s2[at];
    }
#pragma unroll
    for (int i = 0; i < STEPS; ++i) {
        const int at = i * THREADS + static_cast<int>(threadIdx.x);
        if (at < PAIRS) d2[at] = v[i];
    }
}


typedef double mfma_acc_t __attribute__((ext_vector_type(4)));

#ifndef BDG_MFMA_WAVES
#define BDG_MFMA_WAVES 1
#endif

template <int N>
struct MfmaOps {
    using E = Elem<N>;
    static constexpr int MT = (E::Np + 15) / 16;
    static constexpr int KV = (E::Np + 3) / 4;
    static constexpr int KS = (E::NFN + 3) / 4;
    static constexpr int OFF_DR = 0;
    static constexpr int OFF_DS = MT * KV * 64;
    static constexpr int OFF_LIFT = 2 * MT * KV * 64;
    static constexpr int DOUBLES = OFF_LIFT + MT * KS * 64;
};

template <int N, int MODE, bool HALO = false, bool SYNC = false, int THREADS = 256>
__global__ __launch_bounds__(THREADS, (N <= 4 ? 2 : BDG_MFMA_WAVES)) void sw2d_stage_mfma_kernel(const StageParams p) {
    constexpr unsigned WAVES = THREADS / 64;
    using E = Elem<N>;
    using O = MfmaOps<N>;
    constexpr int Np = E::Np, Nfp = E::Nfp, NFN = E::NFN, MT = O::MT, KV = O::KV, KS = O::KS;

    extern __shared__ double sOps[];
    stage_image<O::DOUBLES, THREADS>(sOps, p.opsAffine);
    __syncthreads();

    const unsigned lane = threadIdx.x & 63u, q = lane >> 4, j = lane & 15u;
    const unsigned nwg = gridDim.x, xcd = blockIdx.x % 8u, q8 = nwg / 8u, r8 = nwg % 8u;
    const unsigned blk = (xcd < r8 ? xcd * (q8 + 1u) : r8 * (q8 + 1u) + (xcd - r8) * q8) + blockIdx.x / 8u;
    const unsigned wave = blk * WAVES + (threadIdx.x >> 6), nwaves = nwg * WAVES;
    const unsigned ntiles = (static_cast<unsigned>(p.kend - p.kbegin) + 15u) / 16u;
    const unsigned perWave = (ntiles + nwaves - 1u) / nwaves;
    const unsigned tileEnd = min(ntiles, (wave + 1u) * perWave);

    const long long ld = p.ld, plane = static_cast<long long>(Np) * ld;
    const double* __restrict__ qin = p.qin;
    const double* __restrict__ ag = p.ageo;
    const double g = p.g, halfg = 0.5 * p.g;
    const unsigned kLast = static_cast<unsigned>(p.kend) - 1u;

    bool synced = false;
    for (unsigned tile = wave * perWave; tile < tileEnd; ++tile) {
        if constexpr (SYNC) {
            if (!synced && tile >= static_cast<unsigned>(p.syncFirstTile)) {
                sync_wait(p.syncWait, p.syncWaitValue, p.syncError);
                synced = true;
            }
        }
        const unsigned kTrue = static_cast<unsigned>(p.kbegin) + tile * 16u + j;
        const bool live = kTrue <= kLast;
        const unsigned k = live ? kTrue : kLast;
        const unsigned k8 = k * 8u, k4 = k * 4u;

        int id[KS];
        unsigned mface[KS];
        int fidx[KS];
#pragma unroll
        for (int t = 0; t < KS; ++t) {
            const int jf = 4 * t + static_cast<int>(q), jc = jf < NFN ? jf : 0;
            fidx[t] = jc / Nfp;
            mface[t] = static_cast<unsigned>(fmask_rt<N>(fidx[t], jc - fidx[t] * Nfp));
            id[t] = ld_row(p.vmapP + jc * ld, k4);
        }
        const double rx = ld_row(ag, k8), sx = ld_row(ag + ld, k8), ry = ld_row(ag + 2 * ld, k8), sy = ld_row(ag + 3 * ld, k8);
        const double hf0 = 0.5 * ld_row(ag + 10 * ld, k8), hf1 = 0.5 * ld_row(ag + 11 * ld, k8), hf2 = 0.5 * ld_row(ag + 12 * ld, k8);
        double vh[KV], vhu[KV], vhv[KV];
#pragma unroll
        for (int t = 0; t < KV; ++t) {
            const int m = 4 * t + static_cast<int>(q), mc = m < Np ? m : 0;
            vh[t] = ld_row(qin + mc * ld, k8);
            vhu[t] = ld_row(qin + plane + mc * ld, k8);
            vhv[t] = ld_row(qin + 2 * plane + mc * ld, k8);
        }
        double nxv[KS], nyv[KS], hMv[KS], huMv[KS], hvMv[KS];
#pragma unroll
        for (int t = 0; t < KS; ++t) {
            nxv[t] = ld_row(ag + (4 + fidx[t]) * ld, k8);
            nyv[t] = ld_row(ag + (7 + fidx[t]) * ld, k8);
            hMv[t] = ld_row(qin + static_cast<long long>(mface[t]) * ld, k8);
            huMv[t] = ld_row(qin + plane + static_cast<long long>(mface[t]) * ld, k8);
            hvMv[t] = ld_row(qin + 2 * plane + static_cast<long long>(mface[t]) * ld, k8);
        }
// ... 173 lines not shown
                                        if (sendRec[sr] >= 0)
                                            p.haloSend[static_cast<size_t>(sendRec[sr]) * p.haloRows + c * Np + i] = qn;
                                }
                            } else {
                                const double val = p.ca * oldv[c][r][reg] + p.cb * own + p.cc * R;
                                st_row(p.qout + fo + i * ld, k8, c == 0 ? val : sponge_relax(val, p.sponge));
                            }
                        }
                    }
                }
            }
        }
        if constexpr (SYNC && !HALO) {
            if (tile >= static_cast<unsigned>(p.syncFirstTile)) sync_signal_wave(p.syncSignal);
        }
    }
    if constexpr (SYNC && HALO) sync_signal_workgroup(p.syncSignal);
}

}

namespace bdg_dev {

#ifndef BDG_MFMA2_WAVES
#define BDG_MFMA2_WAVES 2
#endif

template <int N>
struct MfmaOps2 {
    using E = Elem<N>;
    static constexpr int MT = (E::Np + 15) / 16;
    static constexpr int KV = (E::Np + 3) / 4;
    static constexpr int KF = (E::Nfp + 3) / 4;
    static constexpr int OFF_DR = 0;
    static constexpr int OFF_DS = MT * KV * 64;
    static constexpr int OFF_LIFT = 2 * MT * KV * 64;
    static constexpr int DOUBLES = OFF_LIFT + MT * 3 * KF * 64;
};

template <int N, int MODE, int PHYS = 0, bool TRACER = false, bool HALO = false>
__global__ __launch_bounds__(256, BDG_MFMA2_WAVES) void sw2d_stage_mfma2_kernel(const StageParams p, const PhysParams ph) {
    constexpr int NFLD = TRACER ? 4 : 3;
    using E = Elem<N>;
    using O = MfmaOps2<N>;
    constexpr int Np = E::Np, Nfp = E::Nfp, MT = O::MT, KV = O::KV, KF = O::KF;
    constexpr int OFF_F = O::DOUBLES;
    constexpr int IMAGE = O::DOUBLES + (PHYS != 0 ? MT * KV * 64 : 0);

    extern __shared__ double sOps[];
    stage_image<IMAGE, 256>(sOps, p.opsAffine);
    __syncthreads();

    const unsigned lane = threadIdx.x & 63u, q = lane >> 4, j = lane & 15u;
    const unsigned nwg = gridDim.x, xcd = blockIdx.x % 8u, q8 = nwg / 8u, r8 = nwg % 8u;
    const unsigned blk = (xcd < r8 ? xcd * (q8 + 1u) : r8 * (q8 + 1u) + (xcd - r8) * q8) + blockIdx.x / 8u;
    const unsigned wave = blk * 4u + (threadIdx.x >> 6), nwaves = nwg * 4u;
    const unsigned ntiles = (static_cast<unsigned>(p.kend - p.kbegin) + 15u) / 16u;
    const unsigned perWave = (ntiles + nwaves - 1u) / nwaves;
    const unsigned tileEnd = min(ntiles, (wave + 1u) * perWave);

    const long long ld = p.ld, plane = static_cast<long long>(Np) * ld;
    const double* __restrict__ qin = p.qin;
    const double* __restrict__ ag = p.ageo;
    const double g = p.g, halfg = 0.5 * p.g;
    const unsigned kLast = static_cast<unsigned>(p.kend) - 1u;

#pragma unroll 1
    for (unsigned tile = wave * perWave; tile < tileEnd; ++tile) {
        const unsigned kTrue = static_cast<unsigned>(p.kbegin) + tile * 16u + j;
        const bool live = kTrue <= kLast;
        const unsigned k = live ? kTrue : kLast;
        const unsigned k8 = k * 8u, k4 = k * 4u;

        mfma_acc_t acc[NFLD][MT];
#pragma unroll
        for (int c = 0; c < NFLD; ++c)
#pragma unroll
            for (int r = 0; r < MT; ++r) acc[c][r] = mfma_acc_t{0.0, 0.0, 0.0, 0.0};

        int fidx[3][KF];
#pragma unroll
        for (int f = 0; f < 3; ++f)
#pragma unroll
            for (int tf = 0; tf < KF; ++tf) {
                const int n = 4 * tf + static_cast<int>(q);
                fidx[f][tf] = n < Nfp ? ld_row(p.vmapP + (f * Nfp + n) * ld, k4) : 0;
            }

        int btags = 0;
        double lamGlobal = 0.0;
        if constexpr (PHYS == 2) {
            btags = ld_row(ph.obc, k4);
            lamGlobal = *ph.lam;
        }

        {
            const double rx = ld_row(ag, k8), sx = ld_row(ag + ld, k8), ry = ld_row(ag + 2 * ld, k8),
                         sy = ld_row(ag + 3 * ld, k8);
            constexpr int VC = 3, NC = (KV + VC - 1) / VC;
            double hb[2][VC], hub[2][VC], hvb[2][VC];
            double sxb[2][PHYS != 0 ? VC : 1], syb[2][PHYS != 0 ? VC : 1], fcb[2][PHYS != 0 ? VC : 1];
            double hnb[2][TRACER ? VC : 1];
            auto loadChunk = [&](int ch, int buf) {
#pragma unroll
                for (int s = 0; s < VC; ++s) {
                    const int t = ch * VC + s, m = 4 * t + static_cast<int>(q);
                    hb[buf][s] = 1.0; hub[buf][s] = 0.0; hvb[buf][s] = 0.0;
                    if constexpr (PHYS != 0) { sxb[buf][s] = 0.0; syb[buf][s] = 0.0; fcb[buf][s] = ph.fconst; }
// ... 200 lines not shown
                            if (i < Np) {
                                qv[r][reg] = ld_row(qin + fo + i * ld, k8);
                                oldv[r][reg] = ld_row(base2 + i * ld, k8);
                            }
                        }
                    __builtin_amdgcn_sched_barrier(0);
                }
#pragma unroll
                for (int r = 0; r < MT; ++r)
#pragma unroll
                    for (int reg = 0; reg < 4; ++reg) {
                        const int i = 16 * r + static_cast<int>(q) + 4 * reg;
                        if (i < Np) {
                            const double R = acc[c][r][reg];
                            if constexpr (MODE == MODE_RHS) {
                                st_row(p.rhs + fo + i * ld, k8, R);
                            } else if constexpr (MODE == MODE_LSERK) {
                                const double n1 = p.ca * oldv[r][reg] + p.cc * R;
                                const double qn = qv[r][reg] + p.cb * n1;
                                st_row(p.res + fo + i * ld, k8, n1);
                                st_row(p.qout + fo + i * ld, k8, qn);
                                if constexpr (HALO) {
#pragma unroll
                                    for (int sr = 0; sr < 3; ++sr)
                                        if (sendRec[sr] >= 0)
                                            p.haloSend[static_cast<size_t>(sendRec[sr]) * p.haloRows + c * Np + i] = qn;
                                }
                            } else {
                                const double val = p.ca * oldv[r][reg] + p.cb * qv[r][reg] + p.cc * R;
                                double sp = p.sponge;
                                if constexpr (PHYS == 2)
                                    if (ph.spongeField) sp = ld_row(ph.spongeField + i * ld, k8);
                                st_row(p.qout + fo + i * ld, k8, (c == 0 || c == 3) ? val : sponge_relax(val, sp));
                            }
                        }
                    }
                __builtin_amdgcn_sched_barrier(0);
            }
        }
    }
}

template <int N, int MODE>
__global__ __launch_bounds__(256, 3) void sw2d_stage_mfma2_tracer_kernel(const StageParams p) {
    using E = Elem<N>;
    using O = MfmaOps2<N>;
    constexpr int Np = E::Np, Nfp = E::Nfp, MT = O::MT, KV = O::KV, KF = O::KF;

    extern __shared__ double sOps[];
    stage_image<O::DOUBLES, 256>(sOps, p.opsAffine);
    __syncthreads();

    const unsigned lane = threadIdx.x & 63u, q = lane >> 4, j = lane & 15u;
    const unsigned nwg = gridDim.x, xcd = blockIdx.x % 8u, q8 = nwg / 8u, r8 = nwg % 8u;
    const unsigned blk = (xcd < r8 ? xcd * (q8 + 1u) : r8 * (q8 + 1u) + (xcd - r8) * q8) + blockIdx.x / 8u;
    const unsigned wave = blk * 4u + (threadIdx.x >> 6), nwaves = nwg * 4u;
    const unsigned ntiles = (static_cast<unsigned>(p.kend - p.kbegin) + 15u) / 16u;
    const unsigned perWave = (ntiles + nwaves - 1u) / nwaves;
    const unsigned tileEnd = min(ntiles, (wave + 1u) * perWave);

    const long long ld = p.ld, plane = static_cast<long long>(Np) * ld, fo = 3 * plane;
    const double* __restrict__ qin = p.qin;
    const double* __restrict__ ag = p.ageo;
    const double g = p.g;
    const unsigned kLast = static_cast<unsigned>(p.kend) - 1u;

#pragma unroll 1
    for (unsigned tile = wave * perWave; tile < tileEnd; ++tile) {
        const unsigned kTrue = static_cast<unsigned>(p.kbegin) + tile * 16u + j;
        const bool live = kTrue <= kLast;
        const unsigned k = live ? kTrue : kLast;
        const unsigned k8 = k * 8u, k4 = k * 4u;

        mfma_acc_t acc[MT];
#pragma unroll
        for (int r = 0; r < MT; ++r) acc[r] = mfma_acc_t{0.0, 0.0, 0.0, 0.0};
        int fidx[3][KF];
#pragma unroll
        for (int f = 0; f < 3; ++f)
#pragma unroll
            for (int tf = 0; tf < KF; ++tf) {
                const int n = 4 * tf + static_cast<int>(q);
                fidx[f][tf] = n < Nfp ? ld_row(p.vmapP + (f * Nfp + n) * ld, k4) : 0;
            }

        {
            const double rx = ld_row(ag, k8), sx = ld_row(ag + ld, k8), ry = ld_row(ag + 2 * ld, k8),
                         sy = ld_row(ag + 3 * ld, k8);
            constexpr int VC = 3, NC = (KV + VC - 1) / VC;
            double hb[2][VC], hub[2][VC], hvb[2][VC], hnb[2][VC];
            auto loadChunk = [&](int ch, int buf) {
#pragma unroll
                for (int s = 0; s < VC; ++s) {
                    const int t = ch * VC + s, m = 4 * t + static_cast<int>(q);
                    hb[buf][s] = 1.0; hub[buf][s] = 0.0; hvb[buf][s] = 0.0; hnb[buf][s] = 0.0;
                    if (t < KV && m < Np) {
                        hb[buf][s] = ld_row(qin + m * ld, k8);
                        hub[buf][s] = ld_row(qin + plane + m * ld, k8);
                        hvb[buf][s] = ld_row(qin + 2 * plane + m * ld, k8);
                        hnb[buf][s] = ld_row(qin + fo + m * ld, k8);
                    }
                }
            };
            loadChunk(0, 0);
#pragma unroll
            for (int ch = 0; ch < NC; ++ch) {
                const int cur = ch & 1;
                if (ch + 1 < NC) loadChunk(ch + 1, cur ^ 1);
// ... 106 lines not shown
```

### blitzdg_amd/csrc/hip/sw2d_tracer_kernel.hpp

```cpp
#pragma once
#include "sw2d_affine_kernel.hpp"

namespace bdg_dev {

template <int N, int MODE>
__global__ __launch_bounds__(256) void sw2d_stage_tracer_kernel(const StageParams p) {
    using E = Elem<N>;
    constexpr int Np = E::Np, Nfp = E::Nfp, NFN = E::NFN;

    const unsigned nwg = gridDim.x, xcd = blockIdx.x % 8u, q8 = nwg / 8u, r8 = nwg % 8u;
    const unsigned tile = (xcd < r8 ? xcd * (q8 + 1u) : r8 * (q8 + 1u) + (xcd - r8) * q8) + blockIdx.x / 8u;
    const unsigned k = static_cast<unsigned>(p.kbegin) + tile * blockDim.x + threadIdx.x;
    if (k >= static_cast<unsigned>(p.kend)) return;
    const unsigned k8 = k * 8u, k4 = k * 4u;

    const long long ld = p.ld, plane = static_cast<long long>(Np) * ld;
    const double* __restrict__ ops = p.opsAffine;
    const double* __restrict__ qin = p.qin;

    int idx[NFN];
#pragma unroll
    for (int j = 0; j < NFN; ++j) idx[j] = ld_row(p.vmapP + j * ld, k4);
    double h[Np], hu[Np], hv[Np], hN[Np];
#pragma unroll
    for (int n = 0; n < Np; ++n) {
        h[n] = ld_row(qin + n * ld, k8);
        hu[n] = ld_row(qin + plane + n * ld, k8);
        hv[n] = ld_row(qin + 2 * plane + n * ld, k8);
        hN[n] = ld_row(qin + 3 * plane + n * ld, k8);
    }
    const double* __restrict__ ag = p.ageo;
    const double rx = ld_row(ag, k8), sx = ld_row(ag + ld, k8), ry = ld_row(ag + 2 * ld, k8), sy = ld_row(ag + 3 * ld, k8);
    double fnx[3], fny[3], fsc[3];
#pragma unroll
    for (int f = 0; f < 3; ++f) {
        fnx[f] = ld_row(ag + (4 + f) * ld, k8);
        fny[f] = ld_row(ag + (7 + f) * ld, k8);
        fsc[f] = ld_row(ag + (10 + f) * ld, k8);
    }
    __builtin_amdgcn_sched_barrier(0);
    double hP[NFN], huP[NFN], hvP[NFN], hNP[NFN];
#pragma unroll
    for (int j = 0; j < NFN; ++j) {
        const unsigned o8 = static_cast<unsigned>(idx[j] < 0 ? -(idx[j] + 1) : idx[j]) * 8u;
        hP[j] = ld_row(qin, o8);
        huP[j] = ld_row(qin + plane, o8);
        hvP[j] = ld_row(qin + 2 * plane, o8);
        hNP[j] = ld_row(qin + 3 * plane, o8);
    }
    __builtin_amdgcn_sched_barrier(0);

    const double g = p.g;
    double R[Np];
#pragma unroll
    for (int i = 0; i < Np; ++i) R[i] = 0.0;

#pragma unroll
    for (int f = 0; f < 3; ++f) {
        const double nxf = fnx[f], nyf = fny[f];
        double lam = 0.0;
        double uM[Nfp], vM[Nfp], uP[Nfp], vP[Nfp];
#pragma unroll
        for (int n = 0; n < Nfp; ++n) {
            const int j = f * Nfp + n, m = E::fmask(f, n);
// ... 65 lines not shown
```

### blitzdg_amd/csrc/hip/sw2d_vb_kernel.hpp

```cpp
#pragma once
#include "sw2d_affine_kernel.hpp"
#include "sw2d_vd_kernel.hpp"

namespace bdg_dev {

struct VbParams {
    const double* H;
    const double* Hx;
    const double* Hy;
    const int* obc;
    const double* lam;
    const double* sponge;
    double tide;
    double fcor, cd;
    unsigned long long* lamNext;
    double tideNext;
};

struct VbTrace {
    double hM, huM, hvM, hP, huP, hvP, rM, rP;
};

template <int N>
__device__ __forceinline__ VbTrace vb_trace(const double* __restrict__ qin, const double* __restrict__ H,
                                            long long ld, long long plane, unsigned k8, int m, int id, bool open,
                                            double nxf, double nyf, double tide) {
    VbTrace t;
    double hM = ld_row(qin + m * ld, k8);
    double huM = ld_row(qin + plane + m * ld, k8), hvM = ld_row(qin + 2 * plane + m * ld, k8);
    const double HM = ld_row(H + m * ld, k8);
    const unsigned o8 = static_cast<unsigned>(id < 0 ? -(id + 1) : id) * 8u;
    double hP = ld_row(qin, o8);
    double huP = ld_row(qin + plane, o8), hvP = ld_row(qin + 2 * plane, o8);
    const double HP = ld_row(H, o8);
    if (open) {
        huP = huM;
        hvP = hvM;
        hP = HM + tide;
    } else if (id < 0) {
        const double un = huM * nxf + hvM * nyf;
        hP = hM;
        huP = huM - 2 * nxf * un;
        hvP = hvM - 2 * nyf * un;
    }
    const double bM = -HM, bP = -HP, mx = fmax(bP, bM);
    const double hMs = fmax(0.0, hM + bM - mx), hPs = fmax(0.0, hP + bP - mx);
    t.rM = fast_rcp(hMs);
    t.rP = fast_rcp(hPs);
    t.hM = hMs;
    t.hP = hPs;
    t.huM = hMs * (huM * t.rM);
    t.hvM = hMs * (hvM * t.rM);
    t.huP = hPs * (huP * t.rP);
    t.hvP = hPs * (hvP * t.rP);
    return t;
}

template <int N>
__global__ __launch_bounds__(256) void sw2d_vb_speed_kernel(const StageParams p, const VbParams vp,
                                                            double* __restrict__ out) {
    using E = Elem<N>;
    constexpr int Np = E::Np, Nfp = E::Nfp;
    const long long ld = p.ld, plane = static_cast<long long>(Np) * ld;
    const unsigned k = static_cast<unsigned>(p.kbegin) + blockIdx.x * 256u + threadIdx.x;
    double best = 0.0;
    bool bad = false;
    if (k < static_cast<unsigned>(p.kend)) {
        const unsigned k8 = k * 8u, k4 = k * 4u;
        const int tags = ld_row(vp.obc, k4);
#pragma unroll 1
        for (int f = 0; f < 3; ++f) {
            const double nxf = ld_row(p.ageo + (4 + f) * ld, k8), nyf = ld_row(p.ageo + (7 + f) * ld, k8);
            int ids[Nfp];
#pragma unroll
            for (int n = 0; n < Nfp; ++n) ids[n] = ld_row(p.vmapP + (f * Nfp + n) * ld, k4);
#pragma unroll
            for (int n = 0; n < Nfp; ++n) {
                const int j = f * Nfp + n, m = fmask_rt<N>(f, n);
                const int id = ids[n];
                const VbTrace t = vb_trace<N>(p.qin, vp.H, ld, plane, k8, m, id, (tags >> j) & 1, nxf, nyf, vp.tide);
                const double uM = t.huM * t.rM, vM = t.hvM * t.rM, uP = t.huP * t.rP, vP = t.hvP * t.rP;
                const double spdM = sqrt(uM * uM + vM * vM) + sqrt(p.g * t.hM);
                const double spdP = sqrt(uP * uP + vP * vP) + sqrt(p.g * t.hP);
                if (spdM != spdM || spdP != spdP) bad = true;
                best = fmax(best, fmax(spdM, spdP));
            }
        }
    }
    __shared__ double sA[256];
    __shared__ int sBad;
    if (threadIdx.x == 0) sBad = 0;
    __syncthreads();
    if (bad) sBad = 1;
    sA[threadIdx.x] = best;
    __syncthreads();
    for (int s = 128; s > 0; s >>= 1) {
        if (static_cast<int>(threadIdx.x) < s) sA[threadIdx.x] = fmax(sA[threadIdx.x], sA[threadIdx.x + s]);
        __syncthreads();
    }
    if (threadIdx.x == 0) out[blockIdx.x] = sBad ? __builtin_nan("") : sA[0];
}

template <int N>
__global__ __launch_bounds__(256) void sw2d_vb_speed_reduce_kernel(const double* __restrict__ partials, int n,
                                                                   double* __restrict__ out) {
    __shared__ double sA[256];
    __shared__ int sBad;
    if (threadIdx.x == 0) sBad = 0;
    __syncthreads();
    double best = 0.0;
    bool bad = false;
    for (int i = threadIdx.x; i < n; i += 256) {
        const double v = partials[i];
        if (v != v) bad = true;
        best = fmax(best, v);
    }
    if (bad) sBad = 1;
    sA[threadIdx.x] = best;
    __syncthreads();
    for (int s = 128; s > 0; s >>= 1) {
        if (static_cast<int>(threadIdx.x) < s) sA[threadIdx.x] = fmax(sA[threadIdx.x], sA[threadIdx.x + s]);
        __syncthreads();
    }
    if (threadIdx.x == 0) out[0] = sBad ? __builtin_nan("") : sA[0];
}

template <int N, int MODE>
__global__ __launch_bounds__(192, 2) void sw2d_stage_vb_kernel(const StageParams p, const VbParams vp) {
    using E = Elem<N>;
    constexpr int Np = E::Np, Nfp = E::Nfp;

    const unsigned nwg = gridDim.x, xcd = blockIdx.x % 8u, q8 = nwg / 8u, r8 = nwg % 8u;
    const unsigned tile = (xcd < r8 ? xcd * (q8 + 1u) : r8 * (q8 + 1u) + (xcd - r8) * q8) + blockIdx.x / 8u;
    const int c = __builtin_amdgcn_readfirstlane(threadIdx.x >> 6);
    const unsigned k = static_cast<unsigned>(p.kbegin) + tile * 64u + (threadIdx.x & 63u);
    if (k >= static_cast<unsigned>(p.kend)) return;
    const unsigned k8 = k * 8u, k4 = k * 4u;

    const long long ld = p.ld, plane = static_cast<long long>(Np) * ld;
    const double* __restrict__ ops = p.opsAffine;
    const double* __restrict__ qin = p.qin;
    const double* __restrict__ ag = p.ageo;
    const double g = p.g, halfg = 0.5 * p.g;
    const double lam = *vp.lam;

    double R[Np];
#pragma unroll
    for (int i = 0; i < Np; ++i) R[i] = 0.0;

    {
        const double rx = ld_row(ag, k8), sx = ld_row(ag + ld, k8), ry = ld_row(ag + 2 * ld, k8),
                     sy = ld_row(ag + 3 * ld, k8);
#pragma unroll 1
        for (int m = 0; m < Np; ++m) {
            const double h = ld_row(qin + m * ld, k8), hu = ld_row(qin + plane + m * ld, k8),
                         hv = ld_row(qin + 2 * plane + m * ld, k8);
            const double r = fast_rcp(h);
            const double u = hu * r, v = hv * r;
            const double pr = halfg * h * h;
            double F, G;
            if (c == 0) { F = hu; G = hv; }
            else if (c == 1) { F = hu * u + pr; G = hu * v; }
            else { F = hu * v; G = hv * v + pr; }
            const double a = -(rx * F + ry * G), b = -(sx * F + sy * G);
            const double* __restrict__ row = ops + VdOps<N>::OFF_D + 3 * m * Np;
            if (c != 0) {
                const double nrm = fast_sqrt(u * u + v * v);
                double S;
                if (c == 1) S = g * h * ld_row(vp.Hx + m * ld, k8) - vp.cd * u * nrm + vp.fcor * hv;
                else S = g * h * ld_row(vp.Hy + m * ld, k8) - vp.cd * v * nrm - vp.fcor * hu;
#pragma unroll
                for (int i = 0; i < Np; ++i)
                    R[i] = fma(row[3 * i + 2], S, fma(row[3 * i + 1], b, fma(row[3 * i], a, R[i])));
            } else {
#pragma unroll
                for (int i = 0; i < Np; ++i) R[i] = fma(row[3 * i + 1], b, fma(row[3 * i], a, R[i]));
            }
        }
    }

    {
        const int tags = ld_row(vp.obc, k4);
#pragma unroll 1
        for (int f = 0; f < 3; ++f) {
            const double nxf = ld_row(ag + (4 + f) * ld, k8), nyf = ld_row(ag + (7 + f) * ld, k8);
            const double half_fs = 0.5 * ld_row(ag + (10 + f) * ld, k8);
// ... 17 lines not shown
                const double s = half_fs * (dF * nxf + dG * nyf - lam * dq);
                const double* __restrict__ row = ops + VdOps<N>::OFF_LIFT + j * Np;
#pragma unroll
                for (int i = 0; i < Np; ++i) R[i] = fma(row[i], s, R[i]);
            }
        }
    }

    const long long fo = static_cast<long long>(c) * plane;
    if constexpr (MODE == MODE_RHS) {
#pragma unroll
        for (int i = 0; i < Np; ++i) st_row(p.rhs + fo + i * ld, k8, R[i]);
    } else {
        constexpr int CH = 7;
        const double* __restrict__ base2 = ((MODE == MODE_LSERK) ? p.res : p.qbase) + fo;
        const double a = p.ca, b = p.cb, cc = p.cc;
#pragma unroll
        for (int i0 = 0; i0 < Np; i0 += CH) {
            double q1[CH], o1[CH], sp[CH];
#pragma unroll
            for (int t = 0; t < CH; ++t)
                if (i0 + t < Np) {
                    q1[t] = ld_row(qin + fo + (i0 + t) * ld, k8);
                    o1[t] = ld_row(base2 + (i0 + t) * ld, k8);
                    if constexpr (MODE == MODE_COMBINE)
                        sp[t] = (vp.sponge && c != 0) ? ld_row(vp.sponge + (i0 + t) * ld, k8) : p.sponge;
                }
            __builtin_amdgcn_sched_barrier(0);
#pragma unroll
            for (int t = 0; t < CH; ++t) {
                const int i = i0 + t;
                if (i < Np) {
                    if constexpr (MODE == MODE_LSERK) {
                        const double n1 = a * o1[t] + cc * R[i];
                        st_row(p.res + fo + i * ld, k8, n1);
                        st_row(p.qout + fo + i * ld, k8, q1[t] + b * n1);
                    } else {
                        const double val = a * o1[t] + b * q1[t] + cc * R[i];
                        st_row(p.qout + fo + i * ld, k8, c != 0 ? sponge_relax(val, sp[t]) : val);
                    }
                }
            }
            __builtin_amdgcn_sched_barrier(0);
        }
    }
}

template <int N, int MODE, bool FILTERED>
__global__ __launch_bounds__(256) void sw2d_stage_vb_unrolled_kernel(const StageParams p, const VbParams vp,
                                                                      const double* __restrict__ vf) {
    using E = Elem<N>;
    constexpr int Np = E::Np, Nfp = E::Nfp, NFN = E::NFN;

    const unsigned nwg = gridDim.x, xcd = blockIdx.x % 8u, q8 = nwg / 8u, r8 = nwg % 8u;
    const unsigned tile = (xcd < r8 ? xcd * (q8 + 1u) : r8 * (q8 + 1u) + (xcd - r8) * q8) + blockIdx.x / 8u;
    const unsigned k = min(static_cast<unsigned>(p.kbegin) + tile * blockDim.x + threadIdx.x, static_cast<unsigned>(p.kend) - 1u);
    const unsigned k8 = k * 8u, k4 = k * 4u;

    const long long ld = p.ld, plane = static_cast<long long>(Np) * ld;
    const double* __restrict__ ops = p.opsAffine;
    const double* __restrict__ qin = p.qin;
    const double lam = *vp.lam;

    int idx[NFN];
#pragma unroll
    for (int j = 0; j < NFN; ++j) idx[j] = ld_row(p.vmapP + j * ld, k4);
    const int tags = ld_row(vp.obc, k4);
    double h[Np], hu[Np], hv[Np];
#pragma unroll
    for (int n = 0; n < Np; ++n) {
        h[n] = ld_row(qin + n * ld, k8);
        hu[n] = ld_row(qin + plane + n * ld, k8);
        hv[n] = ld_row(qin + 2 * plane + n * ld, k8);
    }
    const double* __restrict__ ag = p.ageo;
    const double rx = ld_row(ag, k8), sx = ld_row(ag + ld, k8), ry = ld_row(ag + 2 * ld, k8), sy = ld_row(ag + 3 * ld, k8);
    double fnx[3], fny[3], fsc[3];
#pragma unroll
    for (int f = 0; f < 3; ++f) {
        fnx[f] = ld_row(ag + (4 + f) * ld, k8);
        fny[f] = ld_row(ag + (7 + f) * ld, k8);
        fsc[f] = ld_row(ag + (10 + f) * ld, k8);
    }
    double HM[NFN], bx[Np], by[Np];
#pragma unroll
    for (int f = 0; f < 3; ++f)
#pragma unroll
        for (int n = 0; n < Nfp; ++n) HM[f * Nfp + n] = ld_row(vp.H + E::fmask(f, n) * ld, k8);
#pragma unroll
    for (int n = 0; n < Np; ++n) {
        bx[n] = ld_row(vp.Hx + n * ld, k8);
        by[n] = ld_row(vp.Hy + n * ld, k8);
    }
    __builtin_amdgcn_sched_barrier(0);
    double hP[NFN], huP[NFN], hvP[NFN], HP[NFN];
#pragma unroll
    for (int j = 0; j < NFN; ++j) {
        const unsigned o8 = static_cast<unsigned>(idx[j] < 0 ? -(idx[j] + 1) : idx[j]) * 8u;
        hP[j] = ld_row(qin, o8);
        huP[j] = ld_row(qin + plane, o8);
        hvP[j] = ld_row(qin + 2 * plane, o8);
        HP[j] = ld_row(vp.H, o8);
    }
    __builtin_amdgcn_sched_barrier(0);

    const double g = p.g, halfg = 0.5 * p.g;
    double R1[Np], R2[Np], R3[Np];
#pragma unroll
// ... 216 lines not shown
```

### blitzdg_amd/csrc/hip/sw2d_vd_kernel.hpp

```cpp
#pragma once
#include "sw2d_affine_kernel.hpp"

namespace bdg_dev {

template <int N>
struct VdOps {
    using E = Elem<N>;
    static constexpr int OFF_D = 0;
    static constexpr int OFF_LIFT = 3 * E::Np * E::Np;
    static constexpr int DOUBLES = OFF_LIFT + E::NFN * E::Np;
};

struct VdParams {
    const double* zx;
    const double* zy;
    const double* fcor;
    double fconst;
    double cd;
    int nf;
    int sources;
    int cbase;
};

template <int N, int MODE>
__global__ __launch_bounds__(256, 2) void sw2d_stage_vd_kernel(const StageParams p, const VdParams vp) {
    using E = Elem<N>;
    constexpr int Np = E::Np, Nfp = E::Nfp;

    const unsigned nwg = gridDim.x, xcd = blockIdx.x % 8u, q8 = nwg / 8u, r8 = nwg % 8u;
    const unsigned tile = (xcd < r8 ? xcd * (q8 + 1u) : r8 * (q8 + 1u) + (xcd - r8) * q8) + blockIdx.x / 8u;
    const int c = __builtin_amdgcn_readfirstlane(threadIdx.x >> 6) + vp.cbase;
    const unsigned k = static_cast<unsigned>(p.kbegin) + tile * 64u + (threadIdx.x & 63u);
    if (k >= static_cast<unsigned>(p.kend)) return;
    const unsigned k8 = k * 8u, k4 = k * 4u;

    const long long ld = p.ld, plane = static_cast<long long>(Np) * ld;
    const double* __restrict__ ops = p.opsAffine;
    const double* __restrict__ qin = p.qin;
    const double* __restrict__ ag = p.ageo;
    const double g = p.g, halfg = 0.5 * p.g;
    const bool tracer = c == 3;
    const bool src = vp.sources != 0 && (c == 1 || c == 2);

    double R[Np];
#pragma unroll
    for (int i = 0; i < Np; ++i) R[i] = 0.0;

    {
        const double rx = ld_row(ag, k8), sx = ld_row(ag + ld, k8), ry = ld_row(ag + 2 * ld, k8),
                     sy = ld_row(ag + 3 * ld, k8);
#pragma unroll 1
        for (int m = 0; m < Np; ++m) {
            const double h = ld_row(qin + m * ld, k8), hu = ld_row(qin + plane + m * ld, k8),
                         hv = ld_row(qin + 2 * plane + m * ld, k8);
            const double r = fast_rcp(h);
            const double u = hu * r, v = hv * r;
            const double pr = halfg * h * h;
            double F, G;
            if (c == 0) { F = hu; G = hv; }
            else if (c == 1) { F = hu * u + pr; G = hu * v; }
            else if (c == 2) { F = hv * u; G = hv * v + pr; }
            else { const double hN = ld_row(qin + 3 * plane + m * ld, k8); F = hN * u; G = hN * v; }
            const double a = -(rx * F + ry * G), b = -(sx * F + sy * G);
            const double* __restrict__ row = ops + VdOps<N>::OFF_D + 3 * m * Np;
            if (src) {
                const double fc = vp.fcor ? ld_row(vp.fcor + m * ld, k8) : vp.fconst;
                const double cdn = vp.cd * fast_sqrt(u * u + v * v);
                double S;
                if (c == 1) {
                    S = fc * hv - cdn * u;
                    if (vp.zx) S -= g * h * ld_row(vp.zx + m * ld, k8);
                } else {
                    S = -(fc * hu - cdn * v);
                    if (vp.zy) S -= g * h * ld_row(vp.zy + m * ld, k8);
                }
#pragma unroll
                for (int i = 0; i < Np; ++i)
                    R[i] = fma(row[3 * i + 2], S, fma(row[3 * i + 1], b, fma(row[3 * i], a, R[i])));
            } else {
#pragma unroll
                for (int i = 0; i < Np; ++i) R[i] = fma(row[3 * i + 1], b, fma(row[3 * i], a, R[i]));
            }
        }
// ... 95 lines not shown
```

### blitzdg_amd/sw2d.py

```python
import weakref

import numpy as np

from . import _capi as C
from ._capi import byref, c_double, c_float, c_int, c_void_p, check, lib
from ._records import RunRecords, locate

REORDER = C.BDG_SW2D_REORDER
NODAL_GEOMETRY = C.BDG_SW2D_NODAL_GEOMETRY
KEEP_ORDER = C.BDG_SW2D_KEEP_ORDER


class Sw2dSolver(RunRecords):

    _abi = "bdg_sw2d"

    def __init__(self, nodes=None, g=9.81, device=0, flags=0, tables=None, fields=3, sources=None):
        h = c_void_p()
        self.fields = int(fields)
        if nodes is not None and (self.fields != 3 or sources is not None):
            ctx = nodes.dgContext()
            tables = {k: getattr(ctx, k) for k in ("Dr", "Ds", "Lift", "rx", "sx", "ry", "sy", "nx", "ny", "Fscale",
                                                   "vmapM", "vmapP")}
            tables["order"] = ctx.order
# ... 145 lines not shown
        if dt is None:
            dt, _ = self.computeDt(CFL)
        tt, dd, st = c_double(t), c_double(dt), c_int()
        check(lib.bdg_sw2d_run_adaptive(self._h, float(CFL), float(finalTime), int(maxSteps), int(bool(filter)),
                                        byref(tt), byref(dd), byref(st)))
        return tt.value, dd.value, st.value

    def synchronize(self):
        check(lib.bdg_sw2d_synchronize(self._h))

    def timeLSERK4Stages(self, dt, nstages):
        ms = c_float()
        check(lib.bdg_sw2d_time_lserk4_stages(self._h, float(dt), int(nstages), byref(ms)))
        return ms.value

    def enableMonitor(self, nodes, H=None, gauges=None, stride=1, capacity=4096):
        w, Hh, el, r, s = self._monitor_inputs(nodes, H, gauges, "TriangleNodesProvisioner")
        rows = C.as_f64(nodes.interpolationRows(r, s), (el.size, self.Np), "rows")
        d = C.Sw2dMonitorDesc(C.ptr(w), C.ptr(Hh), el.size, C.ptr(el) if el.size else None, C.ptr(rows) if el.size else None,
                              int(stride), int(capacity))
        check(lib.bdg_sw2d_enable_monitor(self._h, byref(d)))
        self.numGauges = int(el.size)

    def timeMonitor(self, count):
        ms = c_float()
        check(lib.bdg_sw2d_monitor_time(self._h, int(count), byref(ms)))
        return ms.value

    def enableDrifters(self, nodes, points, mapO=None, stride=1, capacity=1024):
        el, r, s = locate(points, nodes, "points", "TriangleNodesProvisioner")
        vert, neigh, (vinv, jac) = nodes.drifterTables(mapO)
        d = C.Sw2dDrifterDesc(el.size, C.ptr(el), C.ptr(r), C.ptr(s), C.ptr(vert), C.ptr(neigh), C.ptr(vinv), C.ptr(jac),
                              int(stride), int(capacity))
        check(lib.bdg_sw2d_enable_drifters(self._h, byref(d)))
        self.numDrifters = int(el.size)

    def probeStageTraffic(self, repeats=20):
        ms = c_float()
        check(lib.bdg_sw2d_probe_stage_traffic(self._h, int(repeats), byref(ms)))
        return ms.value

    @property
    def isRenumbered(self):
        return bool(lib.bdg_sw2d_is_renumbered(self._h))

    @property
    def usesAffineGeometry(self):
        return bool(lib.bdg_sw2d_uses_affine_geometry(self._h))

    @property
    def deviceBytes(self):
        return lib.bdg_sw2d_device_bytes(self._h)


def streamTriadGBps(device=0, bytesPerArray=1 << 30, repeats=10):
    out = c_double()
    check(lib.bdg_probe_stream_triad(int(device), int(bytesPerArray), int(repeats), byref(out)))
    return out.value


_solver_cache = weakref.WeakKeyDictionary()


def computeRHS(h, hu, hv, g, triangleNodesProvisioner, filter=False, device=0):
    key = triangleNodesProvisioner
    entry = _solver_cache.get(key)
    stamp = (float(g), int(device), getattr(key, "_tables_version", 0))
    if entry is None or entry[0] != stamp:
        entry = (stamp, Sw2dSolver(nodes=key, g=g, device=device))
        _solver_cache[key] = entry
    return entry[1].computeRHS(h, hu, hv, filter=filter)


_script_cache = {}


def sw2dComputeRHS(h, hu, hv, hN, g, H, f, ctx):
    key = (id(ctx), float(g), float(f))
    entry = _script_cache.get(key)
    if entry is None:
        Nfp = int(ctx.numFacePoints)
        tables = {"order": Nfp - 1, "Dr": ctx.Dr, "Ds": ctx.Ds, "Lift": ctx.Lift, "rx": ctx.rx, "sx": ctx.sx,
                  "ry": ctx.ry, "sy": ctx.sy, "nx": ctx.nx, "ny": ctx.ny, "Fscale": ctx.Fscale, "vmapM": ctx.vmapM,
                  "vmapP": ctx.vmapP, "mapW": np.asarray(ctx.BCmap.get(3, []), dtype=np.int32)}
        entry = (Sw2dSolver(tables=tables, g=g, fields=4, sources={"f": float(f), "CD": 0.0}), ctx)
        if len(_script_cache) >= 8:
            _script_cache.pop(next(iter(_script_cache)))
        _script_cache[key] = entry
    return entry[0].computeRHS4(h, hu, hv, hN)
```

### include/blitzdg_hip.h

```cpp
#ifndef BLITZDG_HIP_H
#define BLITZDG_HIP_H

#include <stddef.h>

#ifdef __cplusplus
extern "C" {
#endif

#define BDG_OK 0
#define BDG_ERR_ARGUMENT 1
#define BDG_ERR_RUNTIME 2
#define BDG_ERR_HIP 3
#define BDG_ERR_UNSTABLE 4

typedef struct bdg_mesh bdg_mesh;
typedef struct bdg_trinodes bdg_trinodes;
typedef struct bdg_quadnodes bdg_quadnodes;
typedef struct bdg_nodes1d bdg_nodes1d;
typedef struct bdg_gaussctx bdg_gaussctx;
typedef struct bdg_cubctx bdg_cubctx;
typedef struct bdg_sw2d bdg_sw2d;
typedef struct bdg_sw2dq bdg_sw2dq;

const char* bdg_last_error(void);
// ... 317 lines not shown
    const double* bilinear;
    const int* neighbours;
    const double* bary;
    int stride;
    int capacity;
} bdg_sw2dq_drifter_desc;
int bdg_sw2dq_enable_drifters(bdg_sw2dq* s, const bdg_sw2dq_drifter_desc* desc);
int bdg_sw2dq_drifters_advance(bdg_sw2dq* s, double dt, int num_steps);
int bdg_sw2dq_drifters_time(bdg_sw2dq* s, double dt, int count, float* ms);
int bdg_sw2dq_drifters_state(bdg_sw2dq* s, double* x, double* y, int* element, double* r, double* sref, int* status);
int bdg_sw2dq_drifters_count(const bdg_sw2dq* s, int* num_records, int* num_drifters);
int bdg_sw2dq_drifters_read(bdg_sw2dq* s, int first, int num, double* t, double* x, double* y, int* status);
int bdg_sw2dq_drifters_reset(bdg_sw2dq* s);

int bdg_sw2d_step_lserk4(bdg_sw2d* s, double dt, int num_steps);
int bdg_sw2d_lserk4_stages(bdg_sw2d* s, double dt, int num_stages);
int bdg_sw2d_step_rk2(bdg_sw2d* s, double dt, int num_steps, int filter);
int bdg_sw2d_step_ssprk2(bdg_sw2d* s, double dt, int num_steps, int filter, double sponge_coeff);
int bdg_sw2d_compute_dt(bdg_sw2d* s, double cfl, double* dt, double* eta_max);
int bdg_sw2d_run_adaptive(bdg_sw2d* s, double cfl, double final_time, int max_steps, int filter,
                          double* t_inout, double* dt_inout, int* steps_done);

int bdg_sw2d_set_partition(bdg_sw2d* s, int num_interior, int num_owned, const int* send_elements,
                           int num_send);
int bdg_sw2d_halo_doubles_per_element(const bdg_sw2d* s);
int bdg_sw2d_halo_pack(bdg_sw2d* s, void* send_buffer_device);
int bdg_sw2d_halo_unpack(bdg_sw2d* s, const void* recv_buffer_device);
int bdg_sw2d_lserk4_stage_part(bdg_sw2d* s, double dt, int part);
int bdg_comm_unique_id(void* id_out, int capacity);
int bdg_sw2d_comm_init(bdg_sw2d* s, int rank, int world, const void* unique_id, const int* peer_ranks,
                       const int* send_start, const int* send_count, const int* recv_start,
                       const int* recv_count, int num_peers);
int bdg_sw2d_lserk4_stages_exchanged(bdg_sw2d* s, double dt, int num_stages);
int bdg_sw2d_step_rk2_exchanged(bdg_sw2d* s, double dt, int num_steps, int filter);
int bdg_sw2d_step_ssprk2_exchanged(bdg_sw2d* s, double dt, int num_steps, int filter, double sponge_coeff);
int bdg_sw2d_local_peers(bdg_sw2d* s, int rank, const int* peer_ranks, const int* send_start,
                         const int* send_count, const int* recv_start, const int* recv_count, int num_peers);
int bdg_sw2d_group_lserk4_stages(bdg_sw2d** parts, int num_parts, double dt, int num_stages);
int bdg_sw2d_compute_dt_global(bdg_sw2d* s, double cfl, double* dt, double* eta_max);
int bdg_sw2d_allreduce_max(bdg_sw2d* s, double value, double* out);
int bdg_sw2d_allreduce_sum(bdg_sw2d* s, double value, double* out);
int bdg_sw2d_barrier(bdg_sw2d* s);
int bdg_sw2d_rhs_resident(bdg_sw2d* s, double* rhs1, double* rhs2, double* rhs3);

int bdg_sw2d_synchronize(bdg_sw2d* s);
int bdg_sw2d_time_lserk4_stages(bdg_sw2d* s, double dt, int num_stages, float* ms_per_launch);
int bdg_probe_stream_triad(int device, size_t bytes_per_array, int repeats, double* gbps);
int bdg_sw2d_probe_stage_traffic(bdg_sw2d* s, int repeats, float* ms_per_launch);
int bdg_sw2d_uses_affine_geometry(const bdg_sw2d* s);
int bdg_sw2d_is_renumbered(const bdg_sw2d* s);
int bdg_element_order(const int* EToE, int num_elements, int patch, int* perm);
int bdg_element_order_wanted(const int* EToE, int num_elements, int order);
size_t bdg_sw2d_device_bytes(const bdg_sw2d* s);
void* bdg_sw2d_stream(bdg_sw2d* s);

int bdg_trinodes_quadrature_weights(const bdg_trinodes* nodes, double* w);
int bdg_trinodes_locate_points(const bdg_trinodes* nodes, const double* x, const double* y, int n, int* element, double* r,
                               double* s);
int bdg_trinodes_interpolation_rows(const bdg_trinodes* nodes, const double* r, const double* s, int n, double* rows);
typedef struct bdg_sw2d_monitor_desc {
    const double* weights;
    const double* H;
    int num_gauges;
    const int* gauge_element;
    const double* gauge_row;
    int stride;
    int capacity;
} bdg_sw2d_monitor_desc;
int bdg_sw2d_enable_monitor(bdg_sw2d* s, const bdg_sw2d_monitor_desc* desc);
int bdg_sw2d_monitor_sample(bdg_sw2d* s);
int bdg_sw2d_monitor_count(const bdg_sw2d* s, int* n);
int bdg_sw2d_monitor_read(bdg_sw2d* s, int first, int count, double* records);
int bdg_sw2d_monitor_width(const bdg_sw2d* s, int* width);
int bdg_sw2d_monitor_reset(bdg_sw2d* s);
int bdg_sw2d_monitor_reduce(bdg_sw2d* s);
int bdg_sw2d_monitor_time(bdg_sw2d* s, int count, float* ms);

int bdg_trinodes_drifter_tables(const bdg_trinodes* nodes, const int* mapO, int num_out, double* vertices, int* neighbours,
                                double* vinv, double* jacobi);
typedef struct bdg_sw2d_drifter_desc {
    int count;
    const int* element;
    const double* r;
    const double* s;
    const double* vertices;
    const int* neighbours;
    const double* vinv;
    const double* jacobi;
    int stride;
    int capacity;
} bdg_sw2d_drifter_desc;
int bdg_sw2d_enable_drifters(bdg_sw2d* s, const bdg_sw2d_drifter_desc* desc);
int bdg_sw2d_drifters_advance(bdg_sw2d* s, double dt, int num_steps);
int bdg_sw2d_drifters_time(bdg_sw2d* s, double dt, int count, float* ms);
int bdg_sw2d_drifters_state(bdg_sw2d* s, double* x, double* y, int* element, double* r, double* sref, int* status);
int bdg_sw2d_drifters_count(const bdg_sw2d* s, int* num_records, int* num_drifters);
int bdg_sw2d_drifters_read(bdg_sw2d* s, int first, int num, double* t, double* x, double* y, int* status);
int bdg_sw2d_drifters_reset(bdg_sw2d* s);

typedef struct bdg_field_stats_desc {
    const double* H;
    int stride;
    int num_periods;
    double periods[4];
    int mean;
    int envelope;
// ... 100 lines not shown
```

Before: 43.85 billion.

## Alternate stage sweep direction each launch to reuse L2/LLC-resident tail data

Adds a sweepBack parameter so consecutive whole-mesh stage launches traverse each XCD's chunk of element tiles in alternating forward and reverse order. The tail of the previous launch's working set, which is still cached, is then touched first by the next launch. This applies across all stage kernel variants, the probe and the vb reduction, and can be disabled with an environment variable. The cost is slightly more index arithmetic per block, plus a risk of mapping errors in the mirrored tile paths.

```diff
diff --git a/blitzdg_amd/_capi.py b/blitzdg_amd/_capi.py
--- a/blitzdg_amd/_capi.py
+++ b/blitzdg_amd/_capi.py
@@ -1,6 +1,6 @@
 import ctypes
 import os
-from ctypes import (POINTER, Structure, byref, c_char_p, c_double, c_float, c_int, c_size_t, c_uint,
+from ctypes import (POINTER, Structure, byref, c_char_p, c_double, c_float, c_int, c_longlong, c_size_t, c_uint,
                     c_ulonglong, c_void_p)
 
 import numpy as np
@@ -310,6 +310,8 @@
     "bdg_element_order": (c_int, [_P, c_int, c_int, _P]),
     "bdg_element_order_wanted": (c_int, [_P, c_int, c_int]),
     "bdg_sw2d_device_bytes": (c_size_t, [_P]),
+    "bdg_stage_tile": (c_uint, [c_uint, c_uint, c_uint]),
+    "bdg_sw2d_backward_launches": (c_longlong, [_P]),
     "bdg_sw2d_stream": (c_void_p, [_P]),
     "bdg_trinodes_quadrature_weights": (c_int, [_P, _P]),
     "bdg_trinodes_locate_points": (c_int, [_P, _P, _P, c_int, _P, _P, _P]),
diff --git a/blitzdg_amd/csrc/hip/sw2d_affine_kernel.hpp b/blitzdg_amd/csrc/hip/sw2d_affine_kernel.hpp
--- a/blitzdg_amd/csrc/hip/sw2d_affine_kernel.hpp
+++ b/blitzdg_amd/csrc/hip/sw2d_affine_kernel.hpp
@@ -73,8 +73,7 @@
     constexpr bool kReadRes = MODE == MODE_LSERK && KIND != STAGE_FIRST;
     constexpr bool kWriteRes = KIND != STAGE_LAST;
 
-    const unsigned nwg = gridDim.x, xcd = blockIdx.x % 8u, q8 = nwg / 8u, r8 = nwg % 8u;
-    const unsigned tile = (xcd < r8 ? xcd * (q8 + 1u) : r8 * (q8 + 1u) + (xcd - r8) * q8) + blockIdx.x / 8u;
+    const unsigned tile = stage_tile(blockIdx.x, gridDim.x, static_cast<unsigned>(p.sweepBack));
     const unsigned k = static_cast<unsigned>(p.kbegin) + tile * blockDim.x + threadIdx.x;
     if (k >= static_cast<unsigned>(p.kend)) return;
     const unsigned k8 = k * 8u, k4 = k * 4u;
@@ -397,8 +396,7 @@
     using E = Elem<N>;
     constexpr int Np = E::Np, Nfp = E::Nfp;
 
-    const unsigned nwg = gridDim.x, xcd = blockIdx.x % 8u, q8 = nwg / 8u, r8 = nwg % 8u;
-    const unsigned tile = (xcd < r8 ? xcd * (q8 + 1u) : r8 * (q8 + 1u) + (xcd - r8) * q8) + blockIdx.x / 8u;
+    const unsigned tile = stage_tile(blockIdx.x, gridDim.x, static_cast<unsigned>(p.sweepBack));
     const unsigned k = static_cast<unsigned>(p.kbegin) + tile * blockDim.x + threadIdx.x;
     if (k >= static_cast<unsigned>(p.kend)) return;
     const unsigned k8 = k * 8u, k4 = k * 4u;
@@ -600,8 +598,7 @@
     constexpr int Np = E::Np, Nfp = E::Nfp;
     static_assert(FIELDS == 1 || FIELDS == 3, "FIELDS is 1 or 3");
 
-    const unsigned nwg = gridDim.x, xcd = blockIdx.x % 8u, q8 = nwg / 8u, r8 = nwg % 8u;
-    const unsigned tile = (xcd < r8 ? xcd * (q8 + 1u) : r8 * (q8 + 1u) + (xcd - r8) * q8) + blockIdx.x / 8u;
+    const unsigned tile = stage_tile(blockIdx.x, gridDim.x, static_cast<unsigned>(p.sweepBack));
     const int c = FIELDS == 3 ? 0 : __builtin_amdgcn_readfirstlane(threadIdx.x >> 6);
     const unsigned k = static_cast<unsigned>(p.kbegin) +
                        (FIELDS == 3 ? tile * 256u + threadIdx.x : tile * 64u + (threadIdx.x & 63u));
diff --git a/blitzdg_amd/csrc/hip/sw2d_affine_lean_kernel.hpp b/blitzdg_amd/csrc/hip/sw2d_affine_lean_kernel.hpp
--- a/blitzdg_amd/csrc/hip/sw2d_affine_lean_kernel.hpp
+++ b/blitzdg_amd/csrc/hip/sw2d_affine_lean_kernel.hpp
@@ -8,8 +8,7 @@
     using E = Elem<N>;
     constexpr int Np = E::Np, Nfp = E::Nfp;
 
-    const unsigned nwg = gridDim.x, xcd = blockIdx.x % 8u, q8 = nwg / 8u, r8 = nwg % 8u;
-    const unsigned tile = (xcd < r8 ? xcd * (q8 + 1u) : r8 * (q8 + 1u) + (xcd - r8) * q8) + blockIdx.x / 8u;
+    const unsigned tile = stage_tile(blockIdx.x, gridDim.x, static_cast<unsigned>(p.sweepBack));
     const unsigned k = static_cast<unsigned>(p.kbegin) + tile * blockDim.x + threadIdx.x;
     if (k >= static_cast<unsigned>(p.kend)) return;
     const unsigned k8 = k * 8u, k4 = k * 4u;
diff --git a/blitzdg_amd/csrc/hip/sw2d_affine_xchg_kernel.hpp b/blitzdg_amd/csrc/hip/sw2d_affine_xchg_kernel.hpp
--- a/blitzdg_amd/csrc/hip/sw2d_affine_xchg_kernel.hpp
+++ b/blitzdg_amd/csrc/hip/sw2d_affine_xchg_kernel.hpp
@@ -10,8 +10,7 @@
     constexpr int Np = E::Np, Nfp = E::Nfp, NFN = E::NFN;
     __shared__ double xs[3 * Np * 64];
 
-    const unsigned nwg = gridDim.x, xcd = blockIdx.x % 8u, q8 = nwg / 8u, r8 = nwg % 8u;
-    const unsigned tile = (xcd < r8 ? xcd * (q8 + 1u) : r8 * (q8 + 1u) + (xcd - r8) * q8) + blockIdx.x / 8u;
+    const unsigned tile = stage_tile(blockIdx.x, gridDim.x, static_cast<unsigned>(p.sweepBack));
     const unsigned base = static_cast<unsigned>(p.kbegin) + tile * 64u, lane = threadIdx.x;
     const unsigned k = base + lane;
     if (k >= static_cast<unsigned>(p.kend)) return;
diff --git a/blitzdg_amd/csrc/hip/sw2d_device.hip b/blitzdg_amd/csrc/hip/sw2d_device.hip
--- a/blitzdg_amd/csrc/hip/sw2d_device.hip
+++ b/blitzdg_amd/csrc/hip/sw2d_device.hip
@@ -102,8 +102,8 @@
 __global__ __launch_bounds__(256) void stage_traffic_probe_kernel(const double* __restrict__ qin, double* __restrict__ qout,
                                                                  double* __restrict__ res, const double* __restrict__ ageo,
                                                                  const int* __restrict__ vmapP, int rows, int idxRows,
-                                                                 long long ld, int K, int readRes, int writeRes) {
-    const unsigned k = blockIdx.x * blockDim.x + threadIdx.x;
+                                                                 long long ld, int K, int readRes, int writeRes, int back) {
+    const unsigned k = (back ? gridDim.x - 1u - blockIdx.x : blockIdx.x) * blockDim.x + threadIdx.x;
     if (k >= static_cast<unsigned>(K)) return;
     double acc = 0.0;
     for (int r = 0; r < 13; ++r) acc += ageo[r * ld + k];
@@ -149,6 +149,10 @@
 bool fullStageTraffic() {
     const char* e = std::getenv("BDG_SW2D_FULL_STAGE_TRAFFIC");
     return e && e[0] != '0';
+}
+bool sweepForward() {
+    const char* e = std::getenv("BDG_SW2D_SWEEP");
+    return e && std::string(e) == "forward";
 }
 bool rolledSources() { return std::getenv("BDG_SW2D_ROLLED_SOURCES") != nullptr; }
 bool eventFence() {
@@ -209,6 +213,12 @@
     bool lamExternal = false;
     DevBuf<double> lamPair;
     int lamSlot = 0;
+    bool sweepAlternates = true;
+    unsigned long long sweepLaunches = 0, backwardLaunches = 0;
+    void nextSweep(bdg_dev::StageParams& p, bool wholeMesh) {
+        p.sweepBack = (wholeMesh && sweepAlternates) ? static_cast<int>(sweepLaunches++ & 1ull) : 0;
+        backwardLaunches += static_cast<unsigned long long>(p.sweepBack);
+    }
     const double* lamStateFor = nullptr;
     double lamTideFor = 0.0;
     double nextEvalTime = 0.0;
@@ -359,9 +369,10 @@
         return N >= 8 ? 244 : 248;
     }
 
-    void launchStage(int mode, bool filter, bdg_dev::StageParams& p, const char* what, hipStream_t on = nullptr) {
+    void launchStage(int mode, bool filter, bdg_dev::StageParams& p, const char* what, hipStream_t on = nullptr, bool wholeMesh = true) {
         if (filter && !hasFilter) throw arg_error("filter requested but the solver was created without a Filter matrix");
         hipStream_t st = on ? on : stream;
+        auto sweep = [&] { nextSweep(p, wholeMesh); };
         AffineVariant variant = affineVariant;
         const int smallPinned = env::smallLaunchPinned();
         const int smallLaunch = (smallPinned >= 0 && p.kbegin == 0) ? smallPinned : kSmallLaunch[N];
@@ -403,27 +414,33 @@
                 lamTideFor = vb.tideNext;
                 lamSlot = nxt;
             }
+            if (ownPass) {
+                sweep();
+                hipCheck(kt->stageVb(mode, p, vb, vbPartials.p, lamBuf.p, true, VbStage::None, nullptr, st), what);
+            }
+            sweep();
             if (fastSources) {
                 p.opsAffine = opsAffine.p;
-                hipCheck(kt->stageVb(mode, p, vb, vbPartials.p, lamBuf.p, ownPass, VbStage::Unrolled, filter ? filterT.p : nullptr, st), what);
+                hipCheck(kt->stageVb(mode, p, vb, vbPartials.p, lamBuf.p, false, VbStage::Unrolled, filter ? filterT.p : nullptr, st), what);
             } else if (mfmaSources) {
-                if (ownPass) hipCheck(kt->stageVb(mode, p, vb, vbPartials.p, lamBuf.p, true, VbStage::None, nullptr, st), what);
                 p.opsAffine = filter ? opsMfma2SrcFiltered.p : opsMfma2Src.p;
                 hipCheck(kt->stageMfma2Src(mode, p, physB(), variantBStateOnce() ? SrcForm::OnceVariantB : SrcForm::VariantB, srcIdentity(filter), st), what);
             } else {
                 p.opsAffine = filter ? opsVdFiltered.p : opsVd.p;
-                hipCheck(kt->stageVb(mode, p, vb, vbPartials.p, lamBuf.p, ownPass, VbStage::Rolled, nullptr, st), what);
+                hipCheck(kt->stageVb(mode, p, vb, vbPartials.p, lamBuf.p, false, VbStage::Rolled, nullptr, st), what);
             }
         } else if (variantD && fastSources) {
             bdg_dev::PhysParams ph = physD();
             ph.fmat = filter ? filterT.p : nullptr;
             p.opsAffine = opsAffine.p;
+            sweep();
             if (nf == 4 && !env::tracerPass()) {
                 hipCheck(kt->stageAffineSrc(mode, p, ph, true, st), what);
             } else {
                 hipCheck(kt->stageAffineSrc(mode, p, ph, false, st), what);
                 if (nf == 4) {
                     p.opsAffine = filter ? opsAffineFiltered.p : opsAffine.p;
+                    sweep();
                     hipCheck(kt->stageTracer(mode, p, st), what);
                 }
             }
@@ -433,6 +450,7 @@
             const bool identity = srcIdentity(filter);
             p.opsAffine = filter ? opsMfma2SrcFiltered.p : opsMfma2Src.p;
             const bool stateOnceSrc = !env::sourcesTwoWave();
+            sweep();
             if (stateOnceSrc && kt->mfma3SrcFields >= nf && !env::tracerPass() && fitsOneDescriptor(nf)) {
                 hipCheck(kt->stageMfma2Src(mode, p, ph, nf == 4 ? SrcForm::OnceSourcesTracer : SrcForm::OnceSources, identity, st), what);
             } else if (stateOnceSrc && kt->mfma3TracerPhase && nf == 4 && !env::tracerPass() && fitsOneDescriptor(4)) {
@@ -440,6 +458,7 @@
             } else if (stateOnceSrc && kt->mfma3SrcFields == 3 && nf == 4 && fitsOneDescriptor(3)) {
                 hipCheck(kt->stageMfma2Src(mode, p, ph, SrcForm::OnceSources, identity, st), what);
                 p.opsAffine = filter ? opsMfma2Filtered.p : opsMfma2.p;
+                sweep();
                 hipCheck(kt->stageMfma2Src(mode, p, ph, SrcForm::TracerPass, false, st), what);
             } else if (nf == 4 && kt->mfmaMT <= 2 && !env::tracerPass()) {
                 hipCheck(kt->stageMfma2Src(mode, p, ph, SrcForm::SourcesTracer, false, st), what);
@@ -447,28 +466,36 @@
                 hipCheck(kt->stageMfma2Src(mode, p, ph, SrcForm::Sources, false, st), what);
                 if (nf == 4) {
                     p.opsAffine = filter ? opsMfma2Filtered.p : opsMfma2.p;
+                    sweep();
                     hipCheck(kt->stageMfma2Src(mode, p, ph, SrcForm::TracerPass, false, st), what);
                 }
             }
         } else if (variantD) {
             p.opsAffine = filter ? opsVdFiltered.p : opsVd.p;
+            sweep();
             hipCheck(kt->stageVd(mode, p, vd, st), what);
         } else if (affine && variant == AffineVariant::Mfma) {
             p.opsAffine = filter ? opsMfmaFiltered.p : opsMfma.p;
+            sweep();
             hipCheck(kt->stageMfma(mode, p, st), what);
         } else if (affine && variant == AffineVariant::Mfma3) {
             p.opsAffine = filter ? opsMfma2Filtered.p : opsMfma2.p;
+            sweep();
             hipCheck(kt->stageMfma3(mode, p, st), what);
         } else if (affine && variant == AffineVariant::Mfma2) {
             p.opsAffine = filter ? opsMfma2Filtered.p : opsMfma2.p;
+            sweep();
             hipCheck(kt->stageMfma2(mode, p, st), what);
         } else if (affine) {
             p.opsAffine = filter ? opsAffineFiltered.p : opsAffine.p;
+            sweep();
             hipCheck(kt->stageAffine(mode, variant, p, st), what);
         } else if (nodalMfma) {
             p.opsAffine = filter ? opsMfma2NodalFilter.p : opsMfma2.p;
+            sweep();
             hipCheck(kt->stageMfma3Nodal(mode, filter, p, st), what);
         } else {
+            sweep();
             hipCheck(kt->stage(mode, filter, p, st), what);
         }
     }
@@ -517,7 +544,7 @@
         p.faceLink = faceLink.p;
         p.stageKind = p.ca == 0.0 ? bdg_dev::STAGE_FIRST : (lastOfStep ? bdg_dev::STAGE_LAST : bdg_dev::STAGE_MID);
         nextEvalTime = lastOfStep ? timeNow + dtStage : timeNow;
-        launchStage(bdg_dev::MODE_LSERK, false, p, "sw2d stage kernel <LSERK>", on);
+        launchStage(bdg_dev::MODE_LSERK, false, p, "sw2d stage kernel <LSERK>", on, part == 2);
         expectRing += signals;
         if (done && !recorded) hipCheck(hipEventRecord(done, on ? on : stream), "hipEventRecord");
         if (part != 0 && advance) lserkStageAdvance(s);
@@ -992,6 +1019,7 @@
     s->uploadRows(d.Fscale, s->fscaleNodal, NFN);
 
     s->affineVariant = s->N <= 4 ? bdg_dev::AffineVariant::Unrolled : bdg_dev::AffineVariant::Mfma3;
+    s->sweepAlternates = !env::sweepForward();
     if (const char* e = env::affineVariantPin()) {
         const int v = std::atoi(e);
         if (v >= 0 && v <= 9) {
@@ -2132,11 +2160,13 @@
         s->use();
         const unsigned grid = static_cast<unsigned>((s->K + 255) / 256);
         const bool links = s->faceLink.p != nullptr;
+        unsigned launches = 0;
         auto launch = [&](int stage) {
             const int last = blitzdg::LSERK4::numStages - 1;
+            const int back = s->sweepAlternates ? static_cast<int>(launches++ & 1u) : 0;
             hipLaunchKernelGGL(bdg_dev::stage_traffic_probe_kernel, dim3(grid), dim3(256), 0, s->stream, s->qcur, s->qalt,
                                s->aux.p, s->ageo.p, links ? s->faceLink.p : s->vmapP.p, 3 * s->Np, links ? 3 : s->NFN, s->ld,
-                               s->K, !links || stage != 0 ? 1 : 0, !links || stage != last ? 1 : 0);
+                               s->K, !links || stage != 0 ? 1 : 0, !links || stage != last ? 1 : 0, back);
         };
         launch(1);
         int i = 0;
@@ -2148,6 +2178,8 @@
 int bdg_sw2d_is_renumbered(const bdg_sw2d* s) { return s ? (s->permHost.empty() ? 0 : 1) : -1; }
 
 size_t bdg_sw2d_device_bytes(const bdg_sw2d* s) { return s ? s->bytes : 0; }
+long long bdg_sw2d_backward_launches(const bdg_sw2d* s) { return s ? static_cast<long long>(s->backwardLaunches) : -1; }
+unsigned bdg_stage_tile(unsigned block, unsigned grid, unsigned back) { return bdg_dev::stage_tile(block, grid, back); }
 void* bdg_sw2d_stream(bdg_sw2d* s) { return s ? static_cast<void*>(s->stream) : nullptr; }
 
 }
diff --git a/blitzdg_amd/csrc/hip/sw2d_kernels.hpp b/blitzdg_amd/csrc/hip/sw2d_kernels.hpp
--- a/blitzdg_amd/csrc/hip/sw2d_kernels.hpp
+++ b/blitzdg_amd/csrc/hip/sw2d_kernels.hpp
@@ -1,5 +1,6 @@
 #pragma once
 #include <hip/hip_runtime.h>
+#include "sw2d_stage_tile.hpp"
 
 namespace bdg_dev {
 
@@ -68,6 +69,7 @@
     int gridCap;
     int tileInterleave;
     int stagger;
+    int sweepBack;
     unsigned long long* phaseClock;
     const unsigned long long* syncWait;
     unsigned long long syncWaitValue;
@@ -117,8 +119,7 @@
     for (int t = threadIdx.x; t < E::LDS_DOUBLES; t += blockDim.x) sOps[t] = p.ops[t];
     __syncthreads();
 
-    const unsigned nwg = gridDim.x, xcd = blockIdx.x % 8u, q8 = nwg / 8u, r8 = nwg % 8u;
-    const unsigned tile = (xcd < r8 ? xcd * (q8 + 1u) : r8 * (q8 + 1u) + (xcd - r8) * q8) + blockIdx.x / 8u;
+    const unsigned tile = stage_tile(blockIdx.x, gridDim.x, static_cast<unsigned>(p.sweepBack));
     const long long k = p.kbegin + static_cast<long long>(tile) * blockDim.x + threadIdx.x;
     if (k >= p.kend) return;
 
diff --git a/blitzdg_amd/csrc/hip/sw2d_mfma3_kernel.hpp b/blitzdg_amd/csrc/hip/sw2d_mfma3_kernel.hpp
--- a/blitzdg_amd/csrc/hip/sw2d_mfma3_kernel.hpp
+++ b/blitzdg_amd/csrc/hip/sw2d_mfma3_kernel.hpp
@@ -59,20 +59,22 @@
     const int sBase = IMAGE + static_cast<int>(threadIdx.x >> 6) * Mfma3Lds<N>::TILE_DOUBLES + static_cast<int>(threadIdx.x & 15u);
 
     const unsigned lane = threadIdx.x & 63u, q = lane >> 4, j = lane & 15u;
-    const unsigned nwg = gridDim.x, xcd = blockIdx.x % 8u, q8 = nwg / 8u, r8 = nwg % 8u;
-    const unsigned blk = (xcd < r8 ? xcd * (q8 + 1u) : r8 * (q8 + 1u) + (xcd - r8) * q8) + blockIdx.x / 8u;
+    const unsigned nwg = gridDim.x, wgBefore = stage_chunk_first(blockIdx.x, nwg), wgHere = stage_chunk_length(blockIdx.x, nwg);
+    const unsigned blk = wgBefore + blockIdx.x / 8u;
     const unsigned wave = blk * 4u + (threadIdx.x >> 6), nwaves = nwg * 4u;
     const unsigned ntiles = (static_cast<unsigned>(p.kend - p.kbegin) + 15u) / 16u;
     const unsigned perWave = (ntiles + nwaves - 1u) / nwaves;
     unsigned tileEnd = min(ntiles, (wave + 1u) * perWave), tileStep = 1u;
     unsigned tile = wave * perWave;
+    unsigned xcdLo = min(ntiles, wgBefore * 4u * perWave), xcdHi = min(ntiles, (wgBefore + wgHere) * 4u * perWave);
     if (p.tileInterleave) {
-        const unsigned wgHere = (nwg + 7u - xcd) / 8u, wgBefore = blk - blockIdx.x / 8u;
-        tile = ntiles * wgBefore / nwg + (blockIdx.x / 8u) * 4u + (threadIdx.x >> 6);
-        tileEnd = ntiles * (wgBefore + wgHere) / nwg;
+        tile = xcdLo = ntiles * wgBefore / nwg;
+        tile += (blockIdx.x / 8u) * 4u + (threadIdx.x >> 6);
+        tileEnd = xcdHi = ntiles * (wgBefore + wgHere) / nwg;
         tileStep = wgHere * 4u;
     }
     if (tile >= tileEnd) return;
+    const unsigned back = (SYNC || HALO) ? 0u : static_cast<unsigned>(p.sweepBack);
 
     const long long ld = p.ld, plane = static_cast<long long>(Np) * ld;
     const double g = p.g, halfg = 0.5 * p.g;
@@ -97,7 +99,7 @@
     const __amdgpu_buffer_rsrc_t rrecv = plane_rsrc(HALO ? p.haloRecv : p.ageo, 0xffffffffu);
 
     auto elementOf = [&](unsigned tl, bool& live) {
-        const unsigned kTrue = static_cast<unsigned>(p.kbegin) + tl * 16u + j;
+        const unsigned kTrue = static_cast<unsigned>(p.kbegin) + stage_tile_mirrored(tl, xcdLo, xcdHi, back) * 16u + j;
         live = kTrue <= kLast;
         return live ? kTrue : kLast;
     };
diff --git a/blitzdg_amd/csrc/hip/sw2d_mfma3src_kernel.hpp b/blitzdg_amd/csrc/hip/sw2d_mfma3src_kernel.hpp
--- a/blitzdg_amd/csrc/hip/sw2d_mfma3src_kernel.hpp
+++ b/blitzdg_amd/csrc/hip/sw2d_mfma3src_kernel.hpp
@@ -31,11 +31,10 @@
     const int sBase = IMAGE + static_cast<int>(threadIdx.x >> 6) * L::TILE_DOUBLES + static_cast<int>(threadIdx.x & 15u);
 
     const unsigned lane = threadIdx.x & 63u, q = lane >> 4, j = lane & 15u;
-    const unsigned nwg = gridDim.x, xcd = blockIdx.x % 8u, q8 = nwg / 8u, r8 = nwg % 8u;
-    const unsigned blk = (xcd < r8 ? xcd * (q8 + 1u) : r8 * (q8 + 1u) + (xcd - r8) * q8) + blockIdx.x / 8u;
+    const unsigned nwg = gridDim.x, wgBefore = stage_chunk_first(blockIdx.x, nwg), wgHere = stage_chunk_length(blockIdx.x, nwg);
     const unsigned ntiles = (static_cast<unsigned>(p.kend - p.kbegin) + 15u) / 16u;
-    const unsigned wgHere = (nwg + 7u - xcd) / 8u, wgBefore = blk - blockIdx.x / 8u;
-    unsigned tile = ntiles * wgBefore / nwg + (blockIdx.x / 8u) * 4u + (threadIdx.x >> 6);
+    const unsigned xcdLo = ntiles * wgBefore / nwg;
+    unsigned tile = xcdLo + (blockIdx.x / 8u) * 4u + (threadIdx.x >> 6);
     const unsigned tileEnd = ntiles * (wgBefore + wgHere) / nwg, tileStep = wgHere * 4u;
     if (tile >= tileEnd) return;
 
@@ -60,7 +59,7 @@
     const double cd = ph.cd, slope = ph.slope, dragSign = ph.dragSign, fconst = ph.fconst;
 
     auto elementOf = [&](unsigned tl, bool& live) {
-        const unsigned kTrue = static_cast<unsigned>(p.kbegin) + tl * 16u + j;
+        const unsigned kTrue = static_cast<unsigned>(p.kbegin) + stage_tile_mirrored(tl, xcdLo, tileEnd, static_cast<unsigned>(p.sweepBack)) * 16u + j;
         live = kTrue <= kLast;
         return live ? kTrue : kLast;
     };
diff --git a/blitzdg_amd/csrc/hip/sw2d_mfma_kernel.hpp b/blitzdg_amd/csrc/hip/sw2d_mfma_kernel.hpp
--- a/blitzdg_amd/csrc/hip/sw2d_mfma_kernel.hpp
+++ b/blitzdg_amd/csrc/hip/sw2d_mfma_kernel.hpp
@@ -54,8 +54,8 @@
     __syncthreads();
 
     const unsigned lane = threadIdx.x & 63u, q = lane >> 4, j = lane & 15u;
-    const unsigned nwg = gridDim.x, xcd = blockIdx.x % 8u, q8 = nwg / 8u, r8 = nwg % 8u;
-    const unsigned blk = (xcd < r8 ? xcd * (q8 + 1u) : r8 * (q8 + 1u) + (xcd - r8) * q8) + blockIdx.x / 8u;
+    const unsigned nwg = gridDim.x;
+    const unsigned blk = stage_tile(blockIdx.x, nwg, (HALO || SYNC) ? 0u : static_cast<unsigned>(p.sweepBack));
     const unsigned wave = blk * WAVES + (threadIdx.x >> 6), nwaves = nwg * WAVES;
     const unsigned ntiles = (static_cast<unsigned>(p.kend - p.kbegin) + 15u) / 16u;
     const unsigned perWave = (ntiles + nwaves - 1u) / nwaves;
@@ -335,8 +335,8 @@
     __syncthreads();
 
     const unsigned lane = threadIdx.x & 63u, q = lane >> 4, j = lane & 15u;
-    const unsigned nwg = gridDim.x, xcd = blockIdx.x % 8u, q8 = nwg / 8u, r8 = nwg % 8u;
-    const unsigned blk = (xcd < r8 ? xcd * (q8 + 1u) : r8 * (q8 + 1u) + (xcd - r8) * q8) + blockIdx.x / 8u;
+    const unsigned nwg = gridDim.x;
+    const unsigned blk = stage_tile(blockIdx.x, nwg, HALO ? 0u : static_cast<unsigned>(p.sweepBack));
     const unsigned wave = blk * 4u + (threadIdx.x >> 6), nwaves = nwg * 4u;
     const unsigned ntiles = (static_cast<unsigned>(p.kend - p.kbegin) + 15u) / 16u;
     const unsigned perWave = (ntiles + nwaves - 1u) / nwaves;
@@ -643,8 +643,8 @@
     __syncthreads();
 
     const unsigned lane = threadIdx.x & 63u, q = lane >> 4, j = lane & 15u;
-    const unsigned nwg = gridDim.x, xcd = blockIdx.x % 8u, q8 = nwg / 8u, r8 = nwg % 8u;
-    const unsigned blk = (xcd < r8 ? xcd * (q8 + 1u) : r8 * (q8 + 1u) + (xcd - r8) * q8) + blockIdx.x / 8u;
+    const unsigned nwg = gridDim.x;
+    const unsigned blk = stage_tile(blockIdx.x, nwg, static_cast<unsigned>(p.sweepBack));
     const unsigned wave = blk * 4u + (threadIdx.x >> 6), nwaves = nwg * 4u;
     const unsigned ntiles = (static_cast<unsigned>(p.kend - p.kbegin) + 15u) / 16u;
     const unsigned perWave = (ntiles + nwaves - 1u) / nwaves;
diff --git a/blitzdg_amd/csrc/hip/sw2d_stage_tile.hpp b/blitzdg_amd/csrc/hip/sw2d_stage_tile.hpp
--- /dev/null
+++ b/blitzdg_amd/csrc/hip/sw2d_stage_tile.hpp
@@ -0,0 +1,28 @@
+#pragma once
+
+#if defined(__HIPCC__) || defined(__CUDACC__)
+#define BDG_STAGE_TILE_HD __host__ __device__
+#else
+#define BDG_STAGE_TILE_HD
+#endif
+
+namespace bdg_dev {
+
+BDG_STAGE_TILE_HD inline unsigned stage_chunk_first(unsigned block, unsigned grid) {
+    const unsigned xcd = block % 8u, q8 = grid / 8u, r8 = grid % 8u;
+    return xcd < r8 ? xcd * (q8 + 1u) : r8 * (q8 + 1u) + (xcd - r8) * q8;
+}
+BDG_STAGE_TILE_HD inline unsigned stage_chunk_length(unsigned block, unsigned grid) {
+    return grid / 8u + (block % 8u < grid % 8u ? 1u : 0u);
+}
+
+BDG_STAGE_TILE_HD inline unsigned stage_tile(unsigned block, unsigned grid, unsigned back) {
+    const unsigned at = block / 8u;
+    return stage_chunk_first(block, grid) + (back ? stage_chunk_length(block, grid) - 1u - at : at);
+}
+
+BDG_STAGE_TILE_HD inline unsigned stage_tile_mirrored(unsigned t, unsigned lo, unsigned hi, unsigned back) {
+    return back ? lo + hi - 1u - t : t;
+}
+
+}
diff --git a/blitzdg_amd/csrc/hip/sw2d_tracer_kernel.hpp b/blitzdg_amd/csrc/hip/sw2d_tracer_kernel.hpp
--- a/blitzdg_amd/csrc/hip/sw2d_tracer_kernel.hpp
+++ b/blitzdg_amd/csrc/hip/sw2d_tracer_kernel.hpp
@@ -8,8 +8,7 @@
     using E = Elem<N>;
     constexpr int Np = E::Np, Nfp = E::Nfp, NFN = E::NFN;
 
-    const unsigned nwg = gridDim.x, xcd = blockIdx.x % 8u, q8 = nwg / 8u, r8 = nwg % 8u;
-    const unsigned tile = (xcd < r8 ? xcd * (q8 + 1u) : r8 * (q8 + 1u) + (xcd - r8) * q8) + blockIdx.x / 8u;
+    const unsigned tile = stage_tile(blockIdx.x, gridDim.x, static_cast<unsigned>(p.sweepBack));
     const unsigned k = static_cast<unsigned>(p.kbegin) + tile * blockDim.x + threadIdx.x;
     if (k >= static_cast<unsigned>(p.kend)) return;
     const unsigned k8 = k * 8u, k4 = k * 4u;
diff --git a/blitzdg_amd/csrc/hip/sw2d_vb_kernel.hpp b/blitzdg_amd/csrc/hip/sw2d_vb_kernel.hpp
--- a/blitzdg_amd/csrc/hip/sw2d_vb_kernel.hpp
+++ b/blitzdg_amd/csrc/hip/sw2d_vb_kernel.hpp
@@ -62,7 +62,8 @@
     using E = Elem<N>;
     constexpr int Np = E::Np, Nfp = E::Nfp;
     const long long ld = p.ld, plane = static_cast<long long>(Np) * ld;
-    const unsigned k = static_cast<unsigned>(p.kbegin) + blockIdx.x * 256u + threadIdx.x;
+    const unsigned blk = p.sweepBack ? gridDim.x - 1u - blockIdx.x : blockIdx.x;
+    const unsigned k = static_cast<unsigned>(p.kbegin) + blk * 256u + threadIdx.x;
     double best = 0.0;
     bool bad = false;
     if (k < static_cast<unsigned>(p.kend)) {
@@ -98,7 +99,7 @@
         if (static_cast<int>(threadIdx.x) < s) sA[threadIdx.x] = fmax(sA[threadIdx.x], sA[threadIdx.x + s]);
         __syncthreads();
     }
-    if (threadIdx.x == 0) out[blockIdx.x] = sBad ? __builtin_nan("") : sA[0];
+    if (threadIdx.x == 0) out[blk] = sBad ? __builtin_nan("") : sA[0];
 }
 
 template <int N>
@@ -130,8 +131,7 @@
     using E = Elem<N>;
     constexpr int Np = E::Np, Nfp = E::Nfp;
 
-    const unsigned nwg = gridDim.x, xcd = blockIdx.x % 8u, q8 = nwg / 8u, r8 = nwg % 8u;
-    const unsigned tile = (xcd < r8 ? xcd * (q8 + 1u) : r8 * (q8 + 1u) + (xcd - r8) * q8) + blockIdx.x / 8u;
+    const unsigned tile = stage_tile(blockIdx.x, gridDim.x, static_cast<unsigned>(p.sweepBack));
     const int c = __builtin_amdgcn_readfirstlane(threadIdx.x >> 6);
     const unsigned k = static_cast<unsigned>(p.kbegin) + tile * 64u + (threadIdx.x & 63u);
     if (k >= static_cast<unsigned>(p.kend)) return;
@@ -255,8 +255,7 @@
     using E = Elem<N>;
     constexpr int Np = E::Np, Nfp = E::Nfp, NFN = E::NFN;
 
-    const unsigned nwg = gridDim.x, xcd = blockIdx.x % 8u, q8 = nwg / 8u, r8 = nwg % 8u;
-    const unsigned tile = (xcd < r8 ? xcd * (q8 + 1u) : r8 * (q8 + 1u) + (xcd - r8) * q8) + blockIdx.x / 8u;
+    const unsigned tile = stage_tile(blockIdx.x, gridDim.x, static_cast<unsigned>(p.sweepBack));
     const unsigned k = min(static_cast<unsigned>(p.kbegin) + tile * blockDim.x + threadIdx.x, static_cast<unsigned>(p.kend) - 1u);
     const unsigned k8 = k * 8u, k4 = k * 4u;
 
diff --git a/blitzdg_amd/csrc/hip/sw2d_vd_kernel.hpp b/blitzdg_amd/csrc/hip/sw2d_vd_kernel.hpp
--- a/blitzdg_amd/csrc/hip/sw2d_vd_kernel.hpp
+++ b/blitzdg_amd/csrc/hip/sw2d_vd_kernel.hpp
@@ -27,8 +27,7 @@
     using E = Elem<N>;
     constexpr int Np = E::Np, Nfp = E::Nfp;
 
-    const unsigned nwg = gridDim.x, xcd = blockIdx.x % 8u, q8 = nwg / 8u, r8 = nwg % 8u;
-    const unsigned tile = (xcd < r8 ? xcd * (q8 + 1u) : r8 * (q8 + 1u) + (xcd - r8) * q8) + blockIdx.x / 8u;
+    const unsigned tile = stage_tile(blockIdx.x, gridDim.x, static_cast<unsigned>(p.sweepBack));
     const int c = __builtin_amdgcn_readfirstlane(threadIdx.x >> 6) + vp.cbase;
     const unsigned k = static_cast<unsigned>(p.kbegin) + tile * 64u + (threadIdx.x & 63u);
     if (k >= static_cast<unsigned>(p.kend)) return;
diff --git a/blitzdg_amd/sw2d.py b/blitzdg_amd/sw2d.py
--- a/blitzdg_amd/sw2d.py
+++ b/blitzdg_amd/sw2d.py
@@ -221,6 +221,10 @@
     def deviceBytes(self):
         return lib.bdg_sw2d_device_bytes(self._h)
 
+    @property
+    def backwardLaunches(self):
+        return int(lib.bdg_sw2d_backward_launches(self._h))
+
 
 def streamTriadGBps(device=0, bytesPerArray=1 << 30, repeats=10):
     out = c_double()
diff --git a/include/blitzdg_hip.h b/include/blitzdg_hip.h
--- a/include/blitzdg_hip.h
+++ b/include/blitzdg_hip.h
@@ -393,6 +393,8 @@
 int bdg_element_order(const int* EToE, int num_elements, int patch, int* perm);
 int bdg_element_order_wanted(const int* EToE, int num_elements, int order);
 size_t bdg_sw2d_device_bytes(const bdg_sw2d* s);
+unsigned bdg_stage_tile(unsigned block, unsigned grid, unsigned back);
+long long bdg_sw2d_backward_launches(const bdg_sw2d* s);
 void* bdg_sw2d_stream(bdg_sw2d* s);
 
 int bdg_trinodes_quadrature_weights(const bdg_trinodes* nodes, double* w);
```

New measurement: 45.20 billion (median of 6 runs). 1.03x the previous value.
